# bowen-upenn/scene_graph_commonsense

Measured on AMD Instinct MI355X. Metric: ordered object-pairs/sec (relation head fwd+bwd), batch=8, N=64, higher is better.
Workload: dtype f16 fwd / bf16 bwd (f32 accumulate, f32 master weights); 1 GPU; VG PredCLS synthetic, 8 images x 64 objects per GPU = 32256 ordered pairs per GPU per step, from the raw minibatch; parallelism=dp1

## Files before the change

include/sgc_relhead.h:

```cpp
#ifndef SGC_RELHEAD_H
#define SGC_RELHEAD_H
#ifdef __cplusplus
extern "C" {
#endif


int sgc_pack_image_nhwc(const float* f0, int C0, const float* f1, int C1, void* x_out, int n_img, int HW, int XC, void* stream);

int sgc_conv1_tanh(const void* x, const void* w1r, const float* b1, void* a_img, int n_rows, int XC, void* stream);

int sgc_object_masked_maps(const void* a_img, const int* obj_img, const int* bbox, const void* cst, void* a_pad, int n_obj, int F, int D, void* stream);

int sgc_conv2_object(const void* a_pad, const void* w2r, const float* bias, void* out, int n_obj, void* stream);

int sgc_pair_expand(const void* U, const void* V, const int* sub_idx, const int* obj_idx, void* z_pad, int n_pairs, int out_elem, void* stream);

int sgc_pair_expand_dense(const void* U, const void* V, const int* img_ptr, const int* pid, int pid_ld, int n_img, int max_n,
                          void* z_pad_f16, void* z_pad_bf16, unsigned char* amz, void* stream);
int sgc_pair_expand_dense_windows(const void* U, const void* V, const int* img_ptr, const int* pid, int pid_ld, int n_img, int max_n,
                                  void* z_pad_f16, void* z_pad_bf16, unsigned char* amz, const int* pixel_rect, void* stream);

int sgc_conv3_relu_pool(const void* z_pad, const void* w3r, const float* b3, void* y, unsigned char* argmax, void* y_bf16, int n_pairs,
                        void* stream);

int sgc_shared_windows_count(const int* bbox, const int* sub_idx, const int* obj_idx, int n_pairs, int* count, int* pixel_rect,
                             void* stream);
int sgc_shared_windows_fill(const int* bbox, const int* sub_idx, const int* obj_idx, int n_pairs, const int* count_incl, int* gather,
                            void* stream);
int sgc_conv3_relu_pool_windows(const void* z_pad, const void* w3r, const float* b3, const int* gather, const int* gather_n,
                                int max_entries, void* y, unsigned char* argmax, void* y_bf16, void* stream);
int sgc_shared_windows_assemble(const int* bbox, const int* sub_idx, const int* obj_idx, int n_pairs, int n_obj, const void* y_obj,
                                const unsigned char* argmax_obj, const void* y_obj_bf16, void* y, unsigned char* argmax, void* y_bf16,
                                void* stream);

int sgc_conv2_regions_count(const int* bbox, int n_obj, int* count, void* stream);
int sgc_conv2_regions_fill(const int* bbox, int n_obj, const int* count_incl, int* gather, void* stream);
int sgc_conv2_object_regions(const void* a_pad, const void* w2r, const float* bias, const int* gather, const int* gather_n,
                             int max_entries, void* uv, void* stream);
int sgc_conv2_fill_background(const int* bbox, const int* obj_img, int n_obj, void* uv, void* stream);

int sgc_shared_windows_count3(const int* bbox, const int* sub_idx, const int* obj_idx, int n_pairs, int* count_all, int* count_conv,
                              int* count_linear, int* pixel_rect_conv, void* stream);
int sgc_shared_windows_fill_class(const int* bbox, const int* sub_idx, const int* obj_idx, int n_pairs, const int* count_incl, int* gather,
                                  int cls, void* stream);
int sgc_conv3_windows_raw(const void* z_pad, const void* w3r, const int* gather, const int* gather_n, int max_entries, float* raw,
                          void* stream);
int sgc_conv3_relu_pool_windows_wm_raw(const void* z_pad, const void* w3r, const float* b3, const int* gather, const int* gather_n,
                                       const int* dest, int max_entries, void* ywm, unsigned char* argmax, void* ywm_bf16, float* raw,
                                       int raw_first, void* stream);
int sgc_windows_linear_forward(const int* bbox, const int* sub_idx, const int* obj_idx, const int* obj_img, int n_obj, int n_real_pairs,
                               const int* gather_linear, const int* n_linear, int max_linear, const int* count_incl_all,
                               const int* dest_all, const float* raw, long n_object_entries, const float* b3, void* ywm, void* ywm_bf16,
                               unsigned char* argmax, int* dest_linear, void* stream);
int sgc_windows_linear_backward_objects(const int* bbox, const int* sub_idx, const int* obj_idx, const int* sub_ptr, const int* sub_list,
                                        const int* obj_ptr, const int* obj_list, int n_obj, int n_real_pairs, const int* gather_conv,
                                        int first_object_entry, int n_object_entries, const int* count_incl_all, const int* dest_all,
                                        const void* dywm, const unsigned char* argmax, void* dy3x, void* stream);
int sgc_windows_linear_backward_bg(const int* gather_linear, const int* dest_linear, const int* order, const int* segments, int n_img,
                                   const void* dywm, const unsigned char* argmax, void* dy3_bg_pad, float* bias_part, void* stream);

int sgc_shared_windows_assemble_bwd(const int* bbox, const int* sub_idx, const int* obj_idx, const int* sub_ptr, const int* sub_list,
                                    const int* obj_ptr, const int* obj_list, int n_obj, const void* dy, void* dy_obj, void* stream);
int sgc_windows_unpool(const void* dy, const unsigned char* argmax, const int* gather, const int* gather_n, const int* dest,
                       int entries_pad, void* dy3x, float* bias_part, int* n_parts, void* stream);
int sgc_windows_im2col(const void* z_pad_bf16, const int* gather, const int* gather_n, int entries_pad, void* zcol, void* stream);
int sgc_windows_wgrad(const void* dy3x, const void* zcol, float* slabs, int rows, int splits, int* n_slabs, void* stream);
int sgc_windows_wgrad_gather(const void* dy3x, const void* z_pad_bf16, const int* gather, float* slabs, int rows, int splits, int* n_slabs,
                             void* stream);
int sgc_windows_im2patch(const void* z_pad_bf16, const int* gather, const int* gather_n, int entries_pad, void* zpatch, void* stream);
int sgc_windows_im2patch_f16(const void* z_pad_f16, const int* gather, const int* gather_n, int entries_pad, void* zpatch, void* stream);
int sgc_windows_wgrad_patch(const void* dy3x, const void* zpatch, float* slabs, int rows, int splits, int* n_slabs, void* stream);
int sgc_windows_wgrad_patch_sparse(const void* dywm, const unsigned char* argmax, const int* gather, const int* dest, int n_entries,
                                   const void* zpatch, void* pack_ac, void* pack_ic, float* slabs, int splits, int* n_slabs, void* stream);
int sgc_windows_wgrad_gather_sparse(const void* dywm, const unsigned char* argmax, const int* gather, const int* dest, int n_entries,
                                    const void* z_pad_f16, void* pack_ac, void* pack_ic, float* slabs, int splits, int* n_slabs, void* stream);
int sgc_windows_im2patch_f16_from(const void* z_pad_f16, const int* gather, const int* gather_n, int e0, int entries, void* zpatch, void* stream);
int sgc_windows_dgrad_cols(const void* dy3x, const void* w3col, void* col, int rows, void* stream);
int sgc_windows_col2im(const void* col, const int* bbox, const int* sub_idx, const int* obj_idx, const int* count_incl, int n_pairs,
                       void* dz, void* stream);
int sgc_windows_dgrad_sparse_weights(const float* conv3_weight, void* w3sp, void* stream);
int sgc_windows_patch_sum2(const void* patch, int n16, const int* bbox, const int* sub_idx, const int* obj_idx, const int* count_incl, int n_pairs,
                           void* dz, void* stream);
int sgc_windows_patch_sum_objects2(const void* patch, int n16, const int* bbox, int n_obj, int n_real, const int* count_incl, void* dz, void* stream);
int sgc_windows_dgrad_sparse_pack(const void* dywm, const unsigned char* argmax, const int* gather, const int* dest, int n_sparse,
                                  void* pack_a, void* pack_i, float* bias_part, int* n_parts, void* stream);
int sgc_windows_dgrad_patches_sparse(const void* pack_a, const void* pack_i, int n_sparse, const void* w3sp, void* patch, void* stream);
int sgc_windows_unpool_from(const void* dy, const unsigned char* argmax, const int* gather, const int* gather_n, const int* dest, int entry0,
                            int entries_pad, void* dy3x, float* bias_part, int* n_parts, void* stream);
int sgc_windows_patch_slots(void);
int sgc_windows_dgrad_patches(const void* dy3x, const void* w3patch, void* patch, int entries, void* stream);
int sgc_windows_patch_sum(const void* patch, const int* bbox, const int* sub_idx, const int* obj_idx, const int* count_incl, int n_pairs,
                          void* dz, void* stream);
int sgc_windows_patch_sum_objects(const void* patch, const int* bbox, int n_obj, int n_real_pairs, const int* count_incl, void* dz, void* stream);
int sgc_pair_contract_windows(const void* dz, const unsigned char* amz, const int* ptr, const int* list, const int* pixel_rect,
                              const int* img_ptr, int role, int n_real_pairs, int n_obj, int n_img, int bg_maps, void* dU_pad, void* stream);
int sgc_shared_objects_count(const int* bbox, int n_obj, int* count, int* pixel_rect, void* stream);
int sgc_shared_objects_fill(const int* bbox, int n_obj, int n_real_pairs, const int* count_incl, int* gather, void* stream);
int sgc_shared_objects_fill_rows(const int* bbox, const int* obj_img, int n_obj, const int* goff, const void* y_bg, const void* y_bg_bf16,
                                 const unsigned char* argmax_bg, void* ywm, void* ywm_bf16, unsigned char* argmax_ps, void* stream);
int sgc_shared_objects_bg_grad(const int* bbox, const int* img_ptr, int n_obj, int n_img, const int* goff, const void* dywm, void* dy_bg,
                               void* stream);
int sgc_windows_col2im_objects(const void* col, const int* bbox, int n_obj, int n_real_pairs, const int* count_incl, void* dz, void* stream);

int sgc_conv3_relu_pool_wm(const void* z_pad, const void* w3r, const float* b3, const int* goff, void* ywm, unsigned char* argmax,
                           void* ywm_bf16, int n_pairs, void* stream);
int sgc_conv3_relu_pool_windows_wm(const void* z_pad, const void* w3r, const float* b3, const int* gather, const int* gather_n,
                                   const int* dest, int max_entries, void* ywm, unsigned char* argmax, void* ywm_bf16, void* stream);
int sgc_fc1_products_pitch(void);
int sgc_fc1_windows_gemm(const void* ywm, const void* w1p, const int* tile_group, float* owm, int rows, void* stream);
int sgc_fc1_integral(const float* owm, const int* goff, int n_pseudo, float* S, void* stream);
int sgc_fc1_own_rect_sums(const float* S, const int* bbox, int n_obj, float* own, void* stream);
int sgc_fc1_assemble(const float* S, const float* owm, const int* bbox, const int* sub_idx, const int* obj_idx, const int* count_incl,
                     const int* dest, int n_obj, const float* bias, int drop_enable, unsigned drop_seed, void* h1, int n_pairs,
                     const float* own_rect_sums , void* stream);
int sgc_fc1_assemble_ordered(const float* S, const float* owm, const int* bbox, const int* sub_idx, const int* obj_idx, const int* count_incl,
                             const int* dest, int n_obj, const float* bias, int drop_enable, unsigned drop_seed, void* h1, int n_pairs,
                             const float* own_rect_sums, const int* pair_order, void* stream);
int sgc_fc1_windows_gemm_x16(const void* ywm, const void* w1p, const int* tile_group, const int* goff, int n_pseudo, float* owm, void* oxh,
                             int rows, void* stream);
int sgc_fc1_assemble_x16(const float* S, const void* oxh, const int* bbox, const int* sub_idx, const int* obj_idx, const int* count_incl,
                         const int* dest, int n_obj, const float* bias, int drop_enable, unsigned drop_seed, void* h1, int n_pairs,
                         const float* own_rect_sums, const int* pair_order, void* stream);

int sgc_fc1_gsum(const void* dh1, const int* bbox, const int* sub_idx, const int* obj_idx, const int* sub_ptr, const int* sub_list,
                 const int* obj_ptr, const int* obj_list, const int* goff, int n_obj, void* gwm, void* stream);
int sgc_fc1_xrows(const void* dh1, const int* gather, const int* dest, int n_entries, const int* goff, const int* gend, void* gwm,
                  void* ywm_bf16, void* stream);
int sgc_fc1_windows_dgrad(const void* gwm, const void* w1pT, const int* tile_group, void* dywm, int rows, void* stream);
int sgc_fc1_windows_wgrad(const void* gwm, const void* ywm_bf16, const int* goff, float* dw, int rows, void* stream);

int sgc_window_rows_compact(const int* bbox, const int* obj_img, int n_obj, int n_img, const int* goff, int* prow, void* stream);
int sgc_window_rows_objects_compact(const int* codes, int n, const int* prow, int n_pairs, int* dest, void* stream);
int sgc_shared_objects_fill_argmax(const int* bbox, const int* obj_img, int n_obj, const unsigned char* argmax_bg, unsigned char* argmax_ps,
                                   void* stream);
int sgc_fc1_integral_rows(const float* owm, const int* prow, int n_pseudo, float* S, void* stream);
int sgc_fc1_gsum_groups(int n_obj, int n_img);
int sgc_fc1_gsum_compact(const void* dh1, const int* bbox, const int* sub_idx, const int* obj_idx, const int* sub_ptr, const int* sub_list,
                         const int* obj_ptr, const int* obj_list, const int* img_ptr, int n_img, const int* goff, const int* prow, int n_obj,
                         void* gwm, float* part, void* stream);
int sgc_shared_objects_bg_grad_compact(int n_img, const int* goff, const void* dywm, void* dy_bg, void* stream);

int sgc_fc1_relu(const void* y, const void* w1p, const float* b, void* h1, int n_pairs, int K, int drop_enable, unsigned drop_seed, void* stream);

int sgc_fc2_labels_relu(const void* h1, const void* w2m, const float* b, const float* lsub, const float* lobj, const int* sub_idx,
                        const int* obj_idx, float* p_out, int n_pairs, int drop_enable, unsigned drop_seed, void* stream);

int sgc_bayes_head(const float* p, const float* Wt, const float* bias, int n_pairs, int ng, int np, int ns, int hier, float T1, float T2,
                   float T3, float* rel, float* sup, float* conn, float* cand_conf, int* cand_pred, const unsigned char* iou_mask, void* stream);

int sgc_bayes_head_any(const float* h, const float* W, const float* bias, int M, int D, int ng, int np, int ns, float T1, float T2,
                       float T3, float* rel, float* sup, void* stream);
int sgc_bayes_head_any_bwd(const float* h, const float* W, const float* rel, const float* sup, const float* g_rel, const float* g_sup,
                           int M, int D, int ng, int np, int ns, float T1, float T2, float T3, float* dh, float* part, void* stream);
int sgc_bayes_head_any_wreduce(const float* part, int n_part, int D, float* out, void* stream);
int sgc_bayes_head_any_loss(const float* h, const float* W, const float* bias, const void* target, int target_is_int64,
                            const float* class_weight, int M, int D, int ng, int np, int ns, float T1, float T2, float T3, float* norm,
                            float* dz, double* loss_part, float* loss, void* stream);
int sgc_bayes_head_any_loss_bwd(const float* h, const float* W, const float* dz, const float* g, int M, int D, float* dh, float* part,
                                void* stream);
int sgc_bayes_head_any_candidates(const float* h, const float* W, const float* bias, int M, int D, int ng, int np, int ns, float T1,
                                  float T2, float T3, float* cand_conf, int* cand_pred, float* sup, void* stream);
int sgc_bayes_head_any_loss_cs(const float* h, const float* W, const float* bias, const void* target, int target_is_int64,
                               const float* class_weight, const void* subject_cat, const void* object_cat, int cat_is_int64,
                               const unsigned* aligned, const unsigned* violated, int C, int M, int D, int ng, int np, int ns, float T1,
                               float T2, float T3, float lambda_cs, float lambda_weak, float lambda_strong, float* norm, float* dz,
                               float* dir, unsigned char* flags, double* part, int* cnt_part, float* out, long long* counts,
                               void* stream);
int sgc_bayes_head_any_loss_cs_bwd(const float* h, const float* W, const float* dz, const float* dir, const unsigned char* flags,
                                   const float* coef, const float* g, int M, int D, int ng, int np, int ns, float* dh, float* part,
                                   void* stream);
int sgc_bayes_head_any_candidates_cs(const float* h, const float* W, const float* bias, const void* subject_cat, const void* object_cat,
                                     int cat_is_int64, const unsigned* aligned, const unsigned* violated, int C, int M, int D, int ng,
                                     int np, int ns, float T1, float T2, float T3, float* cand_conf, int* cand_pred, float* sup,
                                     void* stream);

int sgc_topk_per_image(const float* conf, const int* seg_ptr, int n_img, int K, int* out_idx, int* out_count, void* stream);

int sgc_scene_graph_topk(const float* cand_conf, const int* cand_pred, int rep, const float* cat_conf, const float* conn,
                         const unsigned char* mask, const unsigned char* included, const int* image_ptr, const int* pair_list,
                         const int* sub_idx, const int* obj_idx, const long* cats, const unsigned* aligned, const unsigned* violated,
                         int C, int R, int n_img, int K, int slot_major, int* out_pair, int* out_slot, int* out_pred, int* out_sub,
                         int* out_obj, float* out_score, int* out_count, int* out_finite, void* stream);

int sgc_recall_hits(const long* c_scat, const long* c_ocat, const long* c_pred, int n_pred, const float* c_sbox, const float* c_obox,
                    const int* keep_pos, const int* keep_cnt, int K, const int* t_row, const long* t_rel, const long* t_scat,
                    const long* t_ocat, const float* t_sbox, const float* t_obox, int n_targets, const unsigned char* equiv, int n_equiv,
                    int feature_size, double iou_thresh, int* hit, void* stream);

int sgc_related_topk(const long* c_scat, const long* c_ocat, const long* c_pred, const float* c_sbox, const float* c_obox,
                     const float* c_conf, int n_cand, const int* keep_pos, const int* keep_cnt, int K, int top_k, const int* t_ptr,
                     const long* t_scat, const long* t_ocat, const float* t_sbox, const float* t_obox, int n_img, int* out_pos,
                     int* out_rank, int* out_count, float* out_conf, void* stream);

int sgc_recall_accumulate(const int* out_pair, const int* out_pred, const int* out_sub, const int* out_obj, const int* out_count,
                          int n_img, int K, const int* cand_pred, int n_pred, const long* cats, const float* boxes, int n_obj,
                          const int* sub_idx, const int* obj_idx, const int* image, const int* directed,
                          const unsigned char* included, int n_pairs, const int* img_targets, const int* top_k, int n_k,
                          const unsigned* zero_shot, int C, int R, int feature_size, double iou_thresh, long* hits, long* hits_pc,
                          long* targets, long* targets_pc, long* zs_hits, long* zs_hits_pc, long* zs_targets, long* zs_targets_pc,
                          void* stream);

int sgc_recall_accumulate_targets(const int* out_pred, const int* out_sub, const int* out_obj, const int* out_count, int n_img, int K,
                                  const long* cats, const float* boxes, int n_obj, const int* t_image, const long* t_rel,
                                  const long* t_scat, const long* t_ocat, const float* t_sbox, const float* t_obox, int n_targets,
                                  const unsigned char* equiv, int n_equiv, const int* top_k, int n_k, const unsigned* zero_shot, int C,
                                  int R, int feature_size, double iou_thresh, long* hits, long* hits_pc, long* targets,
                                  long* targets_pc, long* zs_hits, long* zs_hits_pc, long* zs_targets, long* zs_targets_pc,
                                  void* stream);

int sgc_assign_pair_targets(const int* sub_idx, const int* obj_idx, const int* image, int n_pairs, const int* pid, int pid_ld,
                            const int* img_ptr, const long* cats, const float* boxes, int n_obj, const int* t_ptr, int n_img,
                            const long* t_rel, const long* t_scat, const long* t_ocat, const float* t_sbox, const float* t_obox,
                            int n_targets, const unsigned char* equiv, int n_equiv, int R, int feature_size, double iou_thresh,
                            int* directed, int* raw, int* matched, int* target_hit, void* stream);

int sgc_precision_accumulate(const int* out_pred, const int* out_sub, const int* out_obj, const int* out_count, int n_img, int K,
                             int n_rank, const int* image_ptr, const int* pair_list, const long* cats, const float* boxes, int n_obj,
                             const int* sub_idx, const int* obj_idx, const int* directed, const unsigned char* included, int n_pairs,
                             int R, int feature_size, double iou_thresh, long* ap, long* ap_union, long* num_ap, void* stream);

int sgc_overlap_filter(const int* bbox, const int* sub_idx, const int* obj_idx, unsigned char* out, int n_pairs, void* stream);

int sgc_commonsense_filter(const long* scat, const long* pred, const long* ocat, float* conf, int n, const unsigned* aligned,
                           const unsigned* violated, int C, int R, void* stream);

int sgc_commonsense_flags(const long* scat, const long* ocat, const int* cand_pred, int n_pairs, int n_cand, const unsigned* aligned,
                          const unsigned* violated, int C, int R, float* weak, float* strong, void* stream);


int sgc_scene_tables(const int* n_per_img, const int* img_ptr, const int* goff, int n_img, int max_n, int n_pairs, int n_obj, int pid_ld,
                     const int* rel_tri, const float* dir_tri, int* sub_idx, int* obj_idx, int* step, int* image, int* directed,
                     int* raw, int* pid, int* obj_ptr, int* sub_list, int* obj_list, int* obj_img, int* step_ptr, void* stream);

int sgc_bucket_place(const int* codes, int n, const int* sub_idx, const int* obj_img, int img_key, int n_keys, const int* base, int* out,
                     int* seg, int mode, void* stream);
long sgc_bucket_place_scratch_ints(int n, int n_keys);
int sgc_bucket_place_seg(const int* codes, int n, const int* sub_idx, const int* obj_img, int img_key, int n_keys, const int* base, int* out,
                         int* seg, int mode, int* scratch, long scratch_ints, void* stream);

int sgc_pseudo_pair_tables(const int* obj_img, int n_obj, int n_img, int n_pairs, int with_bg, int* ps_sub, int* ps_obj, int* bg_codes,
                           int* bg_n, void* stream);

int sgc_scan_rows(const int* in, int* out, int rows, int n, void* stream);

int sgc_window_rows_objects(const int* codes, int n, const int* goff, int n_pairs, int* dest, void* stream);
int sgc_window_rows_conv(const int* codes_conv, int n, const int* incl_conv, const int* incl_all, const int* dest_all, int* dest_conv,
                         void* stream);

int sgc_loss_coefficients(const int* step_ptr, int n_steps, const int* directed, const float* class_weight, int ng, int np, int hier,
                          double lambda_connectivity, double lambda_not_connected, int* tgt, float* coef_a, float* coef_b, float* coef_c,
                          float* conn_y, void* stream);

int sgc_connectivity_stats(const float* conn, const int* directed, const int* raw, const unsigned char* included, int n_pairs,
                           unsigned long long* out5, void* stream);

int sgc_label_vectors(const float* fc2_weight, int ld, int col0, const long* cats, const float* super_multihot, int n_obj, int C, int S,
                      float* lsub, float* lobj, void* stream);
int sgc_label_grads(const float* dlsub, const float* dlobj, const long* cats_sub, const long* cats_obj, const float* mh_sub,
                    const float* mh_obj, int n_obj, int C, int S, float* grad_fc2_weight, int ld, int col0, void* stream);


int sgc_pair_expand_train(const void* U, const void* V, const int* sub_idx, const int* obj_idx, void* z_pad_f16, void* z_pad_bf16,
                          unsigned char* amz, int n_pairs, void* stream);

int sgc_head_loss_bwd(const float* rel, const float* sup, const float* conn, const float* p, const int* tgt, const float* coef_a,
                      const float* coef_b, const float* coef_c, const float* conn_y, const float* W, int n_pairs, int ng, int np, int ns,
                      int hier, float T1, float T2, float T3, float drop_scale, float* dl, float* loss, void* dpre, const float* dp_extra,
                      const float* cs_coef, const float* cand_conf, const int* cand_pred, void* stream);
int sgc_head_bwd_upstream(const float* rel, const float* sup, const float* p, const float* g_rel, const float* g_sup, const float* g_conn,
                          const float* g_hidden, const float* W, int n_pairs, int ng, int np, int ns, int hier, float T1, float T2,
                          float T3, float drop_scale, float* dl, void* dpre, void* stream);
int sgc_head_wgrad(const float* dl, const float* p, float* part, int n_pairs, int chunk, void* stream);

int sgc_supcon_hierar(const float* F, const int* labels, int M, float temperature, float grad_scale, float* G, float* loss_rows,
                      float* dF, void* stream);

int sgc_slab_sum(const float* in, float* out, long n, int slabs, int accumulate, void* stream);
int sgc_fill_zero(void* ptr, long nbytes, void* stream);
int sgc_slab_sum_ld(const float* in, float* out, int rows, int cols, long ld_out, int slabs, void* stream);
int sgc_colsum(int elem, const void* X, float* part, long rows, int cols, int row_blocks, void* stream);
int sgc_segment_sum_rows(const void* X, const int* ptr, const int* list, float* out, int n_seg, int cols, void* stream);
int sgc_convert_f16_bf16(const void* in, void* out, long n, void* stream);
int sgc_transpose_cast(const float* src, void* dst, int out_kind, int na, int nb, long sa_s, long sb_s, long ss_i, long sa_d,
                       long sb_d, long ds_j, void* stream);
int sgc_permute_cast(const float* src, void* dst, int out_kind, int ndim, const int* dims, const long* src_strides, const long* dst_strides,
                     long src_off, long dst_off, void* stream);
int sgc_segment_cast(const float* src, void* dst, int out_kind, int rows, int cols, long src_row_stride, long src_col_stride, int n_seg,
                     const long* dst_off, const long* dst_ld, const long* src_off, void* stream);

int sgc_fc2_dgrad(const void* dpre, const void* w2mT, const void* h1, void* dh1, int n_pairs, float drop_scale, void* stream);
int sgc_fc2_wgrad(const void* dpre, const void* h1_bf16, float* slabs, int n_rows, int splits, int* n_slabs, void* stream);
int sgc_fc1_dgrad(const void* dh1, const void* w1pT, void* dy, int n_pairs, int K, void* stream);
int sgc_fc1_wgrad(const void* dh1, const void* y_bf16, float* dw, int n_rows, int K, void* stream);
int sgc_unpool_relu_bwd(const void* dy, const unsigned char* argmax, void* dy3_pad, float* dbias_part, int* n_parts, int n_pairs, void* stream);
int sgc_conv3_dgrad(const void* dy3_pad, const void* wd3, void* dz, int n_pairs, void* stream);
int sgc_conv3_dgrad_pooled(const void* dy, const unsigned char* argmax, const void* wd3, void* dz, int n_pairs, void* stream);
int sgc_conv3_wgrad(const void* dy3_pad, const void* z_pad_bf16, float* slabs, int n_pairs, int splits, int* n_slabs, void* stream);
int sgc_conv3_wgrad_sparse(const void* dy, const unsigned char* argmax, const void* z_pad_bf16, void* pack_ac, void* pack_ic,
                           float* slabs, int n_pairs, int splits, int* n_slabs, void* stream);
int sgc_unpool_relu_bwd_pack(const void* dy, const unsigned char* argmax, void* dy3_pad, float* dbias_part, int* n_parts,
                             void* pack_ac, void* pack_ic, int n_pairs, void* stream);
int sgc_pair_contract(const void* dz, const unsigned char* amz, const int* ptr, const int* list, void* dU_pad, int n_obj, void* stream);
int sgc_conv2_dgrad(const void* dU_pad, const void* wd2, void* da, int n_obj, void* stream);
int sgc_conv2_bwd_regions(const int* bbox, int n_real, int n_objx, int dilate, int* gather, int* n_out, void* stream);
int sgc_conv2_dgrad_regions(const void* dU_pad, const void* wd2, const int* gather, const int* gather_n, int max_entries, void* da,
                            void* stream);
int sgc_conv2_wgrad(const void* dU_pad, const void* a_pad_bf16, float* slabs, int n_obj, int splits, int* n_slabs, void* stream);
int sgc_object_masked_maps_bwd(const void* da, const int* img_ptr, const int* bbox, float* dA, float* dcst_part, int* n_parts, int n_img,
                               int F, int D, void* stream);
int sgc_tanh_bwd(const float* dA, const void* a_img, void* dpre, long n, void* stream);
int sgc_conv1_wgrad(const void* dpre, const void* x_bf16, float* slabs, int n_rows, int XC, int splits, int* n_slabs, void* stream);

int sgc_conv1_dgrad(const void* dpre_a, const void* wt_a, const void* dpre_b, const void* wt_b, float* out0, int C0, float* out1, int C1,
                    int n_img, int HW, int accumulate, void* stream);

int sgc_sgd_momentum_step(float* w, const float* g, float* momentum_buf, long n, float lr, float momentum, float weight_decay,
                          int first_step, void* stream);
int sgc_sgd_fc1_fused(float* w, const float* g_gemm_order, float* momentum_buf, int rows, float lr, float momentum, float weight_decay,
                      int first_step, void* w1p_f16, void* stream);
int sgc_sgd_momentum_multi(int n_tensors, float* const* w, const float* const* g, float* const* momentum_buf, const long* n, float lr,
                           float momentum, float weight_decay, unsigned first_mask, void* stream);

int sgc_detr_candidates(const float* logits, const float* boxes, const int* alp2fre, int n_img, int n_query, int C1, int num_classes,
                        int topk, float feature_size, int* cand_cat, float* cand_conf, float* cand_box, void* stream);
int sgc_nms_per_class(const int* cand_cat, const float* cand_conf, const float* cand_box, int n_img, int n_query, int topk,
                      double iou_threshold, int* out_slot, int* out_count, void* stream);
int sgc_match_boxes_top2(const float* pred_box, const int* pred_ptr, const float* tgt_box, const int* tgt_ptr, int n_img, int max_tgt,
                         int feature_size, int* top_idx, float* top_iou, void* stream);


int sgc_generic_conv1_tanh(const float* feat, const float* depth, long stride_feat, long stride_depth, const int* img, const int* box,
                           const float* w1, const float* b1, int n_pairs, int C, int F, float* a, void* stream);
int sgc_generic_conv3x3_relu_pool(const float* in, const float* w, const float* b, int n_pairs, int S, int Cin, int Cout, float* out,
                                  unsigned char* code, void* stream);
int sgc_generic_conv3x3_bwd(const float* in, const float* w, const float* dout, const unsigned char* code, int n_pairs, int S, int Cin, int Cout,
                            float* dpre, float* din, float* dw, float* db, void* stream);
int sgc_generic_fc1_relu(const float* y, const float* w1, const float* b1, int n_pairs, int Q, int C8, int dropout, unsigned seed, void* h1,
                         void* stream);
int sgc_generic_fc1_bwd(const void* dh1, const float* y, const float* w1, int n_pairs, int Q, int C8, float* dy, float* dw1, float* db1,
                        void* stream);
int sgc_generic_conv1_bwd(const float* feat, const float* depth, long stride_feat, long stride_depth, const int* img, const int* box, const float* a,
                          float* da, int n_pairs, int C, int F, float* dw1, float* db1, void* stream);
int sgc_generic_conv1_dgrad(const float* dpre1, const float* w1, const int* img, const int* box, int n_pairs, int C, int F, float* out0, int C0,
                            float* out1, int C1, int n_img, int accumulate, void* stream);

int sgc_dbg_gemm_nt(int elem, const void* A, const void* B, void* C, int M, int N, int K, long lda, long ldb, long ldc, const float* bias, void* stream);
int sgc_dbg_gemm_nt_ld(const void* A, const void* B, void* C, int M, int N, int K, long lda, long ldb, void* stream);
int sgc_dbg_conv_nt(int elem, const void* A, const void* B, void* C, int n_img, int lgS, int Cin, int N, const float* bias, void* stream);
int sgc_dbg_gemm_tn(int elem, const void* A, const void* B, float* C, int M, int N, int K, long lda, long ldb, int splits, int* slabs, void* stream);
int sgc_dbg_conv_tn(int elem, const void* A, const void* B, float* C, int M, int n_img, int lgS, int Cin, int splits, int* slabs, void* stream);
int sgc_dbg_tr_probe(const int* addr, short* out, void* stream);
int sgc_dbg_mfma_rate(float* out, int blocks, int iters, int mode, void* stream);
int sgc_dbg_smfmac_probe(const void* a, const void* b, const int* idx, float* c, int abid, void* stream);

#ifdef __cplusplus
}
#endif
#endif
```

scene_graph_commonsense_amd/csrc/capi_debug.hip:

```cpp
#include "gemm_nt.h"
#include "gemm_tn.h"

extern "C" {

int sgc_dbg_gemm_nt(int elem, const void* A, const void* B, void* C, int M, int N, int K,
                    long lda, long ldb, long ldc, const float* bias, void* stream) {
    NtParams p{};
    p.A = (const u16*)A; p.B = (const u16*)B; p.C = C; p.M = M; p.N = N; p.K = K;
    p.lda = lda; p.ldb = ldb; p.ldc = ldc; p.bias = bias;
    if (elem == ELEM_F16) return launch_gemm_nt<ELEM_F16, AMODE_PLAIN, EPI_STORE>(p, (hipStream_t)stream);
    return launch_gemm_nt<ELEM_BF16, AMODE_PLAIN, EPI_STORE>(p, (hipStream_t)stream);
}

int sgc_dbg_gemm_nt_ld(const void* A, const void* B, void* C, int M, int N, int K, long lda, long ldb, void* stream) {
    NtParams p{};
    p.A = (const u16*)A; p.B = (const u16*)B; p.C = C; p.M = M; p.N = N; p.K = K;
    p.lda = lda; p.ldb = ldb; p.ldc = N; p.epi_lds = 1;
    if ((N % 256) || (K % 64) || (lda % 8) || (ldb % 8)) return SGC_ERR_ARG;
    return launch_gemm_nt_pp<ELEM_BF16, EPI_STORE>(p, (hipStream_t)stream);
}

int sgc_dbg_conv_nt(int elem, const void* A, const void* B, void* C, int n_img, int lgS, int Cin, int N,
                    const float* bias, void* stream) {
    NtParams p{};
    p.A = (const u16*)A; p.B = (const u16*)B; p.C = C; p.M = n_img << (2 * lgS); p.N = N; p.K = 9 * Cin;
    p.ldb = 9L * Cin; p.ldc = N; p.lgS = lgS; p.Cin = Cin; p.bias = bias;
    if (elem == ELEM_F16) return launch_gemm_nt<ELEM_F16, AMODE_CONV, EPI_STORE>(p, (hipStream_t)stream);
    return launch_gemm_nt<ELEM_BF16, AMODE_CONV, EPI_STORE>(p, (hipStream_t)stream);
}

int sgc_dbg_gemm_tn(int elem, const void* A, const void* B, float* C, int M, int N, int K,
                    long lda, long ldb, int splits, int* slabs, void* stream) {
    TnParams p{};
    p.A = (const u16*)A; p.B = (const u16*)B; p.C = C; p.M = M; p.N = N; p.K = K;
    p.lda = lda; p.ldb = ldb; p.ldc = N; p.slab_stride = (long)M * N;
    int r = (elem == ELEM_F16) ? launch_gemm_tn<ELEM_F16, BMODE_PLAIN>(p, splits, slabs, (hipStream_t)stream)
                               : launch_gemm_tn<ELEM_BF16, BMODE_PLAIN>(p, splits, slabs, (hipStream_t)stream);
    return r;
}

int sgc_dbg_conv_tn(int elem, const void* A, const void* B, float* C, int M, int n_img, int lgS, int Cin,
                    int splits, int* slabs, void* stream) {
    TnParams p{};
    p.A = (const u16*)A; p.B = (const u16*)B; p.C = C; p.M = M; p.N = 9 * Cin; p.K = n_img << (2 * lgS);
    p.lda = M; p.ldc = 9L * Cin; p.slab_stride = (long)M * 9 * Cin; p.lgS = lgS; p.Cin = Cin;
    int r = (elem == ELEM_F16) ? launch_gemm_tn<ELEM_F16, BMODE_CONV>(p, splits, slabs, (hipStream_t)stream)
                               : launch_gemm_tn<ELEM_BF16, BMODE_CONV>(p, splits, slabs, (hipStream_t)stream);
    return r;
}

__global__ void tr_probe_kernel(const int* addr, short* out) {
    __shared__ __attribute__((aligned(16))) short lds[4096];
    for (int i = threadIdx.x; i < 4096; i += 64) lds[i] = (short)i;
    __syncthreads();
    const s16x4 v = __builtin_amdgcn_ds_read_tr16_b64_v4i16(
        (__attribute__((address_space(3))) s16x4*)((char*)lds + addr[threadIdx.x]));
    for (int j = 0; j < 4; ++j) out[threadIdx.x * 4 + j] = v[j];
}
int sgc_dbg_tr_probe(const int* addr, short* out, void* stream) {
    SGC_LAUNCH(tr_probe_kernel, dim3(1), dim3(64), 0, (hipStream_t)stream, addr, out);
    SGC_CHECK_LAUNCH();
    return SGC_OK;
}

__global__ void smfmac_probe_kernel(const u16* a, const u16* b, const int* idx, float* c, int abid) {
    typedef __bf16 bf16x8_t __attribute__((ext_vector_type(8)));
    typedef __bf16 bf16x16_t __attribute__((ext_vector_type(16)));
    const int l = threadIdx.x;
    bf16x8_t av; bf16x16_t bv;
    for (int i = 0; i < 8; ++i) { u16 t = a[l * 8 + i]; av[i] = __builtin_bit_cast(__bf16, t); }
    for (int i = 0; i < 16; ++i) { u16 t = b[l * 16 + i]; bv[i] = __builtin_bit_cast(__bf16, t); }
    f32x16 acc;
    for (int r = 0; r < 16; ++r) acc[r] = 0.f;
    if (abid == 0) acc = __builtin_amdgcn_smfmac_f32_32x32x32_bf16(av, bv, acc, idx[l], 0, 0);
    else if (abid == 1) acc = __builtin_amdgcn_smfmac_f32_32x32x32_bf16(av, bv, acc, idx[l], 0, 1);
    else acc = __builtin_amdgcn_smfmac_f32_32x32x32_bf16(av, bv, acc, idx[l], 1, 0);
    for (int r = 0; r < 16; ++r) c[l * 16 + r] = acc[r];
}
int sgc_dbg_smfmac_probe(const void* a, const void* b, const int* idx, float* c, int abid, void* stream) {
    SGC_LAUNCH(smfmac_probe_kernel, dim3(1), dim3(64), 0, (hipStream_t)stream, (const u16*)a, (const u16*)b, idx, c, abid);
    SGC_CHECK_LAUNCH();
    return SGC_OK;
}

}
template <int mode>
__global__ __launch_bounds__(512, 2) void mfma_rate_kernel(float* out, int iters) {
    typedef __bf16 bf16x8_t __attribute__((ext_vector_type(8)));
    typedef __bf16 bf16x16_t __attribute__((ext_vector_type(16)));
    f32x16 acc[8];
    for (int i = 0; i < 8; ++i) for (int r = 0; r < 16; ++r) acc[i][r] = 0.f;
    bf16x8_t a; bf16x16_t b;
    for (int i = 0; i < 8; ++i) a[i] = (__bf16)(float)(threadIdx.x * 0.001f + i);
    for (int i = 0; i < 16; ++i) b[i] = (__bf16)(float)(threadIdx.x * 0.002f + i);
    const bf16x8_t b8 = __builtin_shufflevector(b, b, 0, 1, 2, 3, 4, 5, 6, 7);
    const int idx = 0x4444;
    for (int it = 0; it < iters; ++it) {
        if (mode == 0) {
#pragma unroll
            for (int i = 0; i < 8; ++i) acc[i] = __builtin_amdgcn_mfma_f32_32x32x16_bf16(a, b8, acc[i], 0, 0, 0);
        } else {
#pragma unroll
            for (int i = 0; i < 8; ++i) acc[i] = __builtin_amdgcn_smfmac_f32_32x32x32_bf16(a, b, acc[i], idx, 0, 0);
        }
    }
    float s = 0.f;
    for (int i = 0; i < 8; ++i) for (int r = 0; r < 16; ++r) s += acc[i][r];
    if (s == 12345.678f) out[0] = s;
}
extern "C" {
int sgc_dbg_mfma_rate(float* out, int blocks, int iters, int mode, void* stream) {
    if (mode == 0) SGC_LAUNCH(mfma_rate_kernel<0>, dim3(blocks), dim3(512), 0, (hipStream_t)stream, out, iters);
    else SGC_LAUNCH(mfma_rate_kernel<1>, dim3(blocks), dim3(512), 0, (hipStream_t)stream, out, iters);
    SGC_CHECK_LAUNCH();
    return SGC_OK;
}

}
```

scene_graph_commonsense_amd/csrc/gemm_nt.h:

```cpp
#pragma once
#include "common.h"
#include <type_traits>

enum { AMODE_PLAIN = 0, AMODE_CONV = 1, AMODE_CONV_GATHER = 2 };
enum { EPI_STORE = 0, EPI_BIAS_TANH = 1, EPI_BIAS_RELU = 2, EPI_POOL = 3, EPI_FC2 = 4, EPI_RELUMASK = 5, EPI_STORE_F32 = 6,
       EPI_STORE_F32T = 7 };

struct NtParams {
    const u16* A; const u16* B; void* C;
    int M, N, K;
    long lda, ldb, ldc;
    int lgS, Cin;
    const float* bias;
    const u16* mask_src;
    const float* lsub; const float* lobj; const int* sub_idx; const int* obj_idx;
    unsigned char* argmax;
    u16* C2;
    float scale;
    unsigned drop_seed; int drop_enable;
    int tiles_m, tiles_n;
    int epi_lds;
    int halo_walk;
    int patch_aligned;
    const u16* Apool; const unsigned char* Acode;
    const int* gather; const int* gather_n;
    const int* dest;
    const int* wm_goff;
    float* raw; int raw_first;
    const int* tile_group; long group_stride;
    u16* Cx; int x_first;
    long seg_stride; int seg_bpad, seg_split;
};

template <int ELEM>
__device__ __forceinline__ f32x16 mfma32(s16x8 a, s16x8 b, f32x16 c) {
    if constexpr (ELEM == ELEM_F16) {
        return __builtin_amdgcn_mfma_f32_32x32x16_f16(__builtin_bit_cast(f16x8, a), __builtin_bit_cast(f16x8, b), c, 0, 0, 0);
    } else {
        return __builtin_amdgcn_mfma_f32_32x32x16_bf16(__builtin_bit_cast(bf16x8, a), __builtin_bit_cast(bf16x8, b), c, 0, 0, 0);
    }
}

__device__ __forceinline__ long conv_row_base(int m, int lgS, int Cin) {
    const int S = 1 << lgS;
    const int img = m >> (2 * lgS);
    const int ml = m & (S * S - 1);
    const int W = ml >> 2, q = ml & 3;
    const int py = W >> (lgS - 1), px = W & ((S >> 1) - 1);
    const int y = 2 * py + (q >> 1), x = 2 * px + (q & 1);
    return ((long)(img * (S + 2) + y) * (S + 2) + x) * Cin;
}

template <int ELEM, int EPI, int TM, int TN, bool GATHER = false>
__device__ __forceinline__ void nt_epilogue(const NtParams& p, f32x16 (&acc)[TM][TN], int m0, int n0, int wr, int wc, int lane, int m_limit = -1) {
    const int M = GATHER ? m_limit : p.M;
    const int h = lane >> 5, cl = lane & 31;
#pragma unroll
    for (int i = 0; i < TM; ++i) {
#pragma unroll
        for (int j = 0; j < TN; ++j) {
            const int col = n0 + wc * TN * 32 + j * 32 + cl;
            const int rbase = m0 + wr * TM * 32 + i * 32;
            const float bias = p.bias ? p.bias[col] : 0.f;
            if constexpr (EPI == EPI_POOL) {
                u16* out = reinterpret_cast<u16*>(p.C);
#pragma unroll
                for (int w = 0; w < 4; ++w) {
                    float v = acc[i][j][4 * w];
                    int am = 0;
#pragma unroll
                    for (int q = 1; q < 4; ++q) {
                        const float t = acc[i][j][4 * w + q];
                        if (t > v) { v = t; am = q; }
                    }
                    v += bias;
                    const int prow = (rbase >> 2) + 2 * w + h;
                    if (prow * 4 < M) {
                        long arow = prow, yrow = prow;
                        if constexpr (GATHER) {
                            arow = p.gather[prow]; yrow = p.dest ? p.dest[prow] : arow;
                            if (p.raw && prow >= p.raw_first) {
#pragma unroll
                                for (int q = 0; q < 4; ++q) p.raw[((long)(prow - p.raw_first) * 4 + q) * p.ldc + col] = acc[i][j][4 * w + q];
                            }
                        }
                        else if (p.wm_goff) yrow = p.wm_goff[prow & 63] + (prow >> 6);
                        if (!(v > 0.f)) { v = 0.f; am = 4; }
                        out[yrow * p.ldc + col] = to_elem<ELEM>(v);
                        if (p.C2) p.C2[yrow * p.ldc + col] = f32_to_bf16_bits(v);
                        if (p.argmax) p.argmax[arow * p.ldc + col] = (unsigned char)am;
                    }
                }
            } else {
#pragma unroll
                for (int r = 0; r < 16; ++r) {
                    const int row = rbase + (r & 3) + 8 * (r >> 2) + 4 * h;
                    if (row >= M) continue;
                    float v = acc[i][j][r];
                    long o = (long)row * p.ldc + col;
                    if constexpr (GATHER && EPI == EPI_STORE)
                        o = ((long)p.gather[row >> 2] * 4 + (row & 3)) * p.ldc + col;
                    if constexpr (EPI == EPI_STORE) {
                        reinterpret_cast<u16*>(p.C)[o] = to_elem<ELEM>(v + bias);
                    } else if constexpr (EPI == EPI_STORE_F32) {
                        reinterpret_cast<float*>(p.C)[o] = v + bias;
                    } else if constexpr (EPI == EPI_BIAS_TANH) {
                        reinterpret_cast<u16*>(p.C)[o] = to_elem<ELEM>(tanhf(v + bias));
                    } else if constexpr (EPI == EPI_BIAS_RELU) {
                        v = fmaxf(v + bias, 0.f);
                        if (p.drop_enable) v = dropout_keep(p.drop_seed, (uint32_t)(row * p.N + col)) ? v * p.scale : 0.f;
                        reinterpret_cast<u16*>(p.C)[o] = to_elem<ELEM>(v);
                    } else if constexpr (EPI == EPI_FC2) {
                        v += bias + p.lsub[(long)p.sub_idx[row] * p.N + col] + p.lobj[(long)p.obj_idx[row] * p.N + col];
                        v = fmaxf(v, 0.f);
                        if (p.drop_enable) v = dropout_keep(p.drop_seed, (uint32_t)(row * p.N + col)) ? v * p.scale : 0.f;
                        reinterpret_cast<float*>(p.C)[o] = v;
                    } else if constexpr (EPI == EPI_RELUMASK) {
                        const float f = from_elem<ELEM_F16>(p.mask_src[o]);
                        reinterpret_cast<u16*>(p.C)[o] = to_elem<ELEM>(f > 0.f ? v * p.scale : 0.f);
                    }
                }
            }
        }
    }
}

__device__ __forceinline__ void nt_epilogue_f32t(const NtParams& p, f32x16 (&acc)[4][2], int m0, int n0, int wr, int wc, int lane) {
    const int h = lane >> 5, cl = lane & 31;
    float* out = reinterpret_cast<float*>(p.C);
    if (!out) return;
    const int g_first = p.Cx ? p.wm_goff[p.tile_group[m0 >> 8]] + p.x_first : 0;
#pragma unroll
    for (int i = 0; i < 4; ++i) {
        const int row = m0 + wr * 128 + i * 32 + cl;
        if (row >= p.M) continue;
        const bool xrow = p.Cx && row >= g_first;
#pragma unroll
        for (int j = 0; j < 2; ++j) {
#pragma unroll
            for (int rq = 0; rq < 4; ++rq) {
                const int col = n0 + wc * 64 + j * 32 + 8 * rq + 4 * h;
                f32x4 v = {acc[i][j][4 * rq], acc[i][j][4 * rq + 1], acc[i][j][4 * rq + 2], acc[i][j][4 * rq + 3]};
                if (p.bias) {
                    const f32x4 b = *reinterpret_cast<const f32x4*>(p.bias + col);
                    v += b;
                }
                if (xrow) {
                    uint2 hv;
                    hv.x = (unsigned)f32_to_f16_bits(v[0]) | ((unsigned)f32_to_f16_bits(v[1]) << 16);
                    hv.y = (unsigned)f32_to_f16_bits(v[2]) | ((unsigned)f32_to_f16_bits(v[3]) << 16);
                    *reinterpret_cast<uint2*>(p.Cx + (long)row * p.N + col) = hv;
                    continue;
                }
                f32x4* dst = reinterpret_cast<f32x4*>(out + (long)row * p.ldc + col);
                *dst = v;
            }
        }
    }
}

__device__ __forceinline__ void supertile_map(int id, int tiles_m, int tiles_n, int& tm, int& tn) {
    constexpr int GS = 16;
    const int a = id / (GS * tiles_n);
    const int hm = min(GS, tiles_m - a * GS);
    const int id2 = id - a * GS * tiles_n;
    const int sn = (tiles_n + GS - 1) / GS;
    const int b = min(id2 / (hm * GS), sn - 1);
    const int id3 = id2 - b * hm * GS;
    const int wn = min(GS, tiles_n - b * GS);
    tm = a * GS + id3 / wn;
    tn = b * GS + id3 % wn;
}

__device__ __forceinline__ void supertile_map_g(int id, int tiles_m, int tiles_n, int GM, int GN, int& tm, int& tn) {
    const int a = id / (GM * tiles_n);
    const int hm = min(GM, tiles_m - a * GM);
    const int id2 = id - a * GM * tiles_n;
    const int sn = (tiles_n + GN - 1) / GN;
    const int b = min(id2 / (hm * GN), sn - 1);
    const int id3 = id2 - b * hm * GN;
    const int wn = min(GN, tiles_n - b * GN);
    tm = a * GM + id3 / wn;
    tn = b * GN + id3 % wn;
}

constexpr int EPI_LDS_PITCH = 128;
constexpr int EPI_LDS_BYTES = 8 * 128 * EPI_LDS_PITCH;
template <int ELEM, bool MASK = false>
__device__ __forceinline__ void nt_epilogue_store16(const NtParams& p, f32x16 (&acc)[4][2], int m0, int n0, int wr, int wc, int lane,
                                                    int wid, char* smem) {
    __syncthreads();
    char* reg = smem + wid * (128 * EPI_LDS_PITCH);
    const int h = lane >> 5, cl = lane & 31;
    const bool odd = cl & 1;
#pragma unroll
    for (int i = 0; i < 4; ++i) {
#pragma unroll
        for (int j = 0; j < 2; ++j) {
            const int col = n0 + wc * 64 + j * 32 + cl;
            const float bias = p.bias ? p.bias[col] : 0.f;
#pragma unroll
            for (int rp = 0; rp < 8; ++rp) {
                float v0 = acc[i][j][2 * rp] + bias, v1 = acc[i][j][2 * rp + 1] + bias;
                if constexpr (MASK) { v0 *= p.scale; v1 *= p.scale; }
                const float recv = __shfl_xor(odd ? v0 : v1, 1);
                const int r0 = ((2 * rp) & 3) + 8 * ((2 * rp) >> 2) + 4 * h;
                const float flo = odd ? recv : v0, fhi = odd ? v1 : recv;
                unsigned packed;
                if constexpr (ELEM == ELEM_BF16) packed = f32x2_to_bf16x2_bits(flo, fhi);
                else packed = (unsigned)to_elem<ELEM>(flo) | ((unsigned)to_elem<ELEM>(fhi) << 16);
                const int row = i * 32 + r0 + (odd ? 1 : 0);
                *reinterpret_cast<unsigned*>(reg + row * EPI_LDS_PITCH + (((j * 32 + (cl & ~1)) * 2) ^ ((row & 1) << 6))) = packed;
            }
        }
    }
    __builtin_amdgcn_wave_barrier();
    u16* out = reinterpret_cast<u16*>(p.C);
    const int c8 = lane & 7, rsub = lane >> 3;
#pragma unroll
    for (int it = 0; it < 16; ++it) {
        const int rowl = it * 8 + rsub;
        uint4 v = *reinterpret_cast<const uint4*>(reg + rowl * EPI_LDS_PITCH + ((c8 * 16) ^ ((rowl & 1) << 6)));
        const int row = m0 + wr * 128 + rowl;
        if (row < p.M) {
            const long o = (long)row * p.ldc + n0 + wc * 64 + c8 * 8;
            if constexpr (MASK) {
                const uint4 f = *reinterpret_cast<const uint4*>(p.mask_src + o);
                const u16* fh = reinterpret_cast<const u16*>(&f);
                u16* vh = reinterpret_cast<u16*>(&v);
#pragma unroll
                for (int k = 0; k < 8; ++k)
                    if (!(from_elem<ELEM_F16>(fh[k]) > 0.f)) vh[k] = 0;
            }
            *reinterpret_cast<uint4*>(out + o) = v;
        }
    }
}

template <int ELEM, int AMODE, int EPI, int WR, int WC, int TM, int TN>
__global__ __launch_bounds__(WR * WC * 64, 2) void gemm_nt_kernel(const NtParams p) {
    extern __shared__ __attribute__((aligned(16))) char smem[];
    constexpr int NW = WR * WC;
    constexpr int BM = WR * TM * 32, BN = WC * TN * 32;
    constexpr int A_BYTES = BM * 128, B_BYTES = BN * 128, BUF_BYTES = A_BYTES + B_BYTES;
    constexpr int AI = BM / (8 * NW), BI = BN / (8 * NW);
    const int tid = threadIdx.x, lane = tid & 63;
    const int wid = __builtin_amdgcn_readfirstlane(tid >> 6);
    int tm, tn;
    supertile_map(blockIdx.x, p.tiles_m, p.tiles_n, tm, tn);
    const int m0 = tm * BM, n0 = tn * BN;
    int Mlim = p.M;
    if constexpr (AMODE == AMODE_CONV_GATHER) {
        Mlim = min(p.M, 4 * *p.gather_n);
        if (m0 >= Mlim) return;
    }

    const int lrow = lane >> 3, cpos = lane & 7;
    const u16* a_ptr[AI];
    const u16* b_ptr[BI];
#pragma unroll
    for (int i = 0; i < AI; ++i) {
        const int row = wid * AI * 8 + i * 8 + lrow;
        const int chunk = cpos ^ ((row >> 1) & 7);
        int m = m0 + row; if (m > Mlim - 1) m = Mlim - 1;
        if constexpr (AMODE == AMODE_CONV_GATHER) m = p.gather[m >> 2] * 4 + (m & 3);
        if constexpr (AMODE != AMODE_PLAIN) a_ptr[i] = p.A + conv_row_base(m, p.lgS, p.Cin) + chunk * 8;
        else a_ptr[i] = p.A + (long)m * p.lda + chunk * 8;
    }
#pragma unroll
    for (int i = 0; i < BI; ++i) {
        const int row = wid * BI * 8 + i * 8 + lrow;
        const int chunk = cpos ^ ((row >> 1) & 7);
        b_ptr[i] = p.B + (long)(n0 + row) * p.ldb + chunk * 8;
    }
    const int Wp = (1 << p.lgS) + 2;

    auto stage = [&](int buf, int kt) {
        long aoff;
        if constexpr (AMODE != AMODE_PLAIN) {
            const int cc = kt / 9, tap = kt - cc * 9;
            const int ky = tap / 3, kx = tap - 3 * ky;
            aoff = (long)(ky * Wp + kx) * p.Cin + (cc << 6);
        } else {
            aoff = (long)kt << 6;
        }
        const long boff = (long)kt << 6;
        char* abase = smem + buf * BUF_BYTES + wid * (AI * 1024);
        char* bbase = smem + buf * BUF_BYTES + A_BYTES + wid * (BI * 1024);
#pragma unroll
        for (int i = 0; i < AI; ++i)
            __builtin_amdgcn_global_load_lds(GLB_PTR(a_ptr[i] + aoff), LDS_PTR(abase + i * 1024), 16, 0, 0);
#pragma unroll
        for (int i = 0; i < BI; ++i)
            __builtin_amdgcn_global_load_lds(GLB_PTR(b_ptr[i] + boff), LDS_PTR(bbase + i * 1024), 16, 0, 0);
    };

    const int wr = wid / WC, wc = wid % WC;
    const int kh = lane >> 5;
    int a_off[TM], a_sw[TM], b_off[TN], b_sw[TN];
#pragma unroll
    for (int i = 0; i < TM; ++i) {
        const int ra = wr * TM * 32 + i * 32 + (lane & 31);
        a_off[i] = ra * 128; a_sw[i] = (ra >> 1) & 7;
    }
#pragma unroll
    for (int i = 0; i < TN; ++i) {
        const int rb = wc * TN * 32 + i * 32 + (lane & 31);
        b_off[i] = rb * 128; b_sw[i] = (rb >> 1) & 7;
    }
    f32x16 acc[TM][TN];
#pragma unroll
    for (int i = 0; i < TM; ++i)
#pragma unroll
        for (int j = 0; j < TN; ++j)
#pragma unroll
            for (int r = 0; r < 16; ++r) acc[i][j][r] = 0.f;

    const int nk = p.K >> 6;
    stage(0, 0);
    for (int kt = 0; kt < nk; ++kt) {
        asm volatile("s_waitcnt vmcnt(0)" ::: "memory");
        __syncthreads();
        if (kt + 1 < nk) stage((kt + 1) & 1, kt + 1);
        const char* ab = smem + (kt & 1) * BUF_BYTES;
        const char* bb = ab + A_BYTES;
#pragma unroll
        for (int ks = 0; ks < 4; ++ks) {
            const int c = ks * 2 + kh;
            s16x8 af[TM], bf[TN];
#pragma unroll
            for (int i = 0; i < TM; ++i) af[i] = *reinterpret_cast<const s16x8*>(ab + a_off[i] + ((c ^ a_sw[i]) << 4));
#pragma unroll
            for (int i = 0; i < TN; ++i) bf[i] = *reinterpret_cast<const s16x8*>(bb + b_off[i] + ((c ^ b_sw[i]) << 4));
#pragma unroll
            for (int i = 0; i < TM; ++i)
#pragma unroll
                for (int j = 0; j < TN; ++j) acc[i][j] = mfma32<ELEM>(af[i], bf[j], acc[i][j]);
        }
    }

    if constexpr (EPI == EPI_STORE && TM == 4 && TN == 2 && WR * WC == 8) {
        if (p.epi_lds) { nt_epilogue_store16<ELEM>(p, acc, m0, n0, wr, wc, lane, wid, smem); return; }
    }
    if constexpr (AMODE == AMODE_CONV_GATHER) nt_epilogue<ELEM, EPI, TM, TN, true>(p, acc, m0, n0, wr, wc, lane, Mlim);
    else nt_epilogue<ELEM, EPI, TM, TN>(p, acc, m0, n0, wr, wc, lane);
}

template <int ELEM, int AMODE, int EPI, int WR, int WC, int TM, int TN>
static int launch_gemm_nt_cfg(NtParams p, hipStream_t stream) {
    constexpr int BM = WR * TM * 32, BN = WC * TN * 32;
    constexpr int LDS0 = 2 * (BM + BN) * 128;
    constexpr int LDS = (EPI == EPI_STORE && TM == 4 && TN == 2 && WR * WC == 8 && LDS0 < EPI_LDS_BYTES) ? EPI_LDS_BYTES : LDS0;
    p.tiles_m = (p.M + BM - 1) / BM;
    p.tiles_n = p.N / BN;
    auto kern = gemm_nt_kernel<ELEM, AMODE, EPI, WR, WC, TM, TN>;
    (void)hipFuncSetAttribute(reinterpret_cast<const void*>(kern), hipFuncAttributeMaxDynamicSharedMemorySize, LDS);
    SGC_LAUNCH(kern, dim3((unsigned)(p.tiles_m * p.tiles_n)), dim3(WR * WC * 64), LDS, stream, p);
    SGC_CHECK_LAUNCH();
    return SGC_OK;
}


#include "gemm_nt_pp.h"

template <int ELEM, int AMODE, int EPI>
static int launch_gemm_nt(NtParams p, hipStream_t stream) {
    static_assert(AMODE == AMODE_PLAIN || AMODE == AMODE_CONV, "gathered rows have their own launchers");
    if (p.M <= 0) return SGC_OK;
    if ((p.K & 63) || (p.N & 127) || p.K <= 0) return SGC_ERR_ARG;
    if (AMODE == AMODE_CONV && ((p.Cin & 63) || p.K != 9 * p.Cin)) return SGC_ERR_ARG;
    p.epi_lds = 1;
    const bool big = (p.N % 256) == 0 && (long)p.M * p.N >= 256L * 256 * 256;
    if constexpr (AMODE == AMODE_CONV && (EPI == EPI_POOL || EPI == EPI_STORE)) {
        if (big && p.lgS == 4 && (p.M % 256) == 0) return launch_conv16_halo_pp<ELEM, EPI>(p, stream);
    }
    if (big) {
        if constexpr (AMODE == AMODE_PLAIN) return launch_gemm_nt_pp<ELEM, EPI>(p, stream);
        else return launch_gemm_nt_cfg<ELEM, AMODE, EPI, 2, 4, 4, 2>(p, stream);
    }
    return launch_gemm_nt_cfg<ELEM, AMODE, EPI, 2, 2, 2, 2>(p, stream);
}
```

scene_graph_commonsense_amd/csrc/gemm_nt_pp.h:

```cpp
#pragma once

#define SGC_WAIT_VM(n) asm volatile("s_waitcnt vmcnt(" #n ")" ::: "memory")
#define SGC_WAIT_LGKM0() asm volatile("s_waitcnt lgkmcnt(0)" ::: "memory")
#define SGC_PP_BARRIER()                                       \
    do {                                                       \
        __builtin_amdgcn_sched_barrier(0);                     \
        __builtin_amdgcn_s_barrier();                          \
        __builtin_amdgcn_sched_barrier(0);                     \
    } while (0)

__device__ __forceinline__ void buf_load_lds16(const void* base, int voff, int soff, void* lds) {
    const __amdgpu_buffer_rsrc_t r = __builtin_amdgcn_make_buffer_rsrc(const_cast<void*>(base), 0, 0x7fffffff, 0x00020000);
    __builtin_amdgcn_raw_ptr_buffer_load_lds(r, LDS_PTR(lds), 16, voff, soff, 0, 0);
}

__device__ __forceinline__ void xcd_patch_map(int id, int tiles_m, int tiles_n, int& tm, int& tn, int gm = 4, int gn = 8) {
    const int nb = tiles_m * tiles_n, q = nb >> 3, r = nb & 7, x = id & 7;
    const int lin = (x < r ? x * (q + 1) : r * (q + 1) + (x - r) * q) + (id >> 3);
    supertile_map_g(lin, tiles_m, tiles_n, gm, gn, tm, tn);
}

__host__ __device__ __forceinline__ int xcd_patch_gn(int tiles_n) { return tiles_n >= 8 ? 8 : (tiles_n >= 4 ? 4 : (tiles_n >= 2 ? 2 : 1)); }
static inline int xcd_patch_grid(int tiles_m, int tiles_n) {
    const int gn = xcd_patch_gn(tiles_n), gm = 32 / gn;
    const int npatch = ((tiles_m + gm - 1) / gm) * ((tiles_n + gn - 1) / gn);
    return ((npatch + 7) / 8) * 8 * 32;
}
__device__ __forceinline__ bool xcd_patch_map_aligned(int id, int tiles_m, int tiles_n, int& tm, int& tn) {
    const int gn = xcd_patch_gn(tiles_n), gm = 32 / gn;
    const int sn = (tiles_n + gn - 1) / gn, npatch = ((tiles_m + gm - 1) / gm) * sn;
    const int x = id & 7, j = id >> 3;
    const int patch = (j >> 5) * 8 + x, w = j & 31;
    if (patch >= npatch) return false;
    const int a = patch / sn, b = patch - a * sn;
    const int wn = min(gn, tiles_n - b * gn);
    tm = a * gm + w / wn;
    tn = b * gn + w % wn;
    return tm < tiles_m && w < gm * wn;
}

template <int ELEM, bool GATHER>
__device__ __forceinline__ void nt_epilogue_pool16(const NtParams& p, f32x16 (&acc)[4][2], int m0, int n0, int wr, int wc, int lane,
                                                   int wid, char* smem, int m_limit);
template <int ELEM, int EPI, int ACG = 0, int SEG = 0>
__global__ __launch_bounds__(512, 2) void gemm_nt_pp_kernel(const NtParams p) {
    extern __shared__ __attribute__((aligned(16))) char smem[];
    constexpr int HT = 16384;
    const int tid = threadIdx.x, lane = tid & 63;
    const int wid = __builtin_amdgcn_readfirstlane(tid >> 6);
    const int wr = wid >> 2, wc = wid & 3;
    int tm, tn;
    if constexpr (SEG) {
        xcd_patch_map(blockIdx.x, p.tiles_m, p.tiles_n, tm, tn, 16, 2);
    } else if (p.patch_aligned) {
        if (!xcd_patch_map_aligned(blockIdx.x, p.tiles_m, p.tiles_n, tm, tn)) return;
    } else {
        xcd_patch_map(blockIdx.x, p.tiles_m, p.tiles_n, tm, tn);
    }
    const int m0 = tm * 256;
    int n0 = tn * 256, n_tile = tn, Kloc = p.K, seg_py = 0, seg_px = 0, seg_ny = 1, seg_nx = 1, seg_c0 = 0;
    long ldb = p.ldb, b_off = 0;
    if constexpr (SEG) {
        const int slot = tn >> 1;
        int pp = 0, part = 0;
        if (p.seg_split) {
            int acc = 0;
            for (pp = 0; pp < 16; ++pp) {
                const int wdt = (((pp >> 2) == 1 || (pp >> 2) == 2) && ((pp & 3) == 1 || (pp & 3) == 2)) ? 2 : 1;
                if (slot < acc + wdt) { part = slot - acc; break; }
                acc += wdt;
            }
        } else {
            pp = slot;
        }
        n_tile = tn & 1;
        n0 = slot * 512 + n_tile * 256;
        seg_py = pp >> 2; seg_px = pp & 3;
        auto cnt1 = [](int c) { return (c == 0 || c == 3) ? 1 : 2; };
        seg_ny = cnt1(seg_py); seg_nx = cnt1(seg_px);
        const int ncomb = seg_ny * seg_nx;
        seg_c0 = (p.seg_split && ncomb == 4) ? 2 * part : 0;
        Kloc = ((p.seg_split && ncomb == 4) ? 2 : ncomb) * 1024;
        ldb = ncomb * 1024 + p.seg_bpad;
        for (int j = 0; j < pp; ++j) b_off += 512L * (1024 * (cnt1(j >> 2) * cnt1(j & 3)) + p.seg_bpad);
        b_off += seg_c0 * 1024;
    }
    int Mlim = p.M;
    long img0 = 0;
    if constexpr (ACG) {
        Mlim = min(p.M, 4 * *p.gather_n);
        if (m0 >= Mlim) return;
        img0 = p.gather[m0 >> 2] >> (2 * p.lgS - 2);
    }
    const int SP = (1 << p.lgS) + 2;
    const long img_elems = (long)SP * SP * p.Cin;

    const int lrow = lane >> 3, cpos = lane & 7;
    const u16* const a_blk = ACG ? p.A + img0 * img_elems : p.A + (long)m0 * p.lda;
    const u16* const b_blk = p.B + b_off + (long)(n_tile * 256) * ldb + (p.tile_group ? (long)p.tile_group[tm] * p.group_stride : 0L);
    int voff[4][2];
#pragma unroll
    for (int q = 0; q < 2; ++q) {
        const int r = (wid * 2 + q) * 8 + lrow;
        const int chunk = (cpos ^ ((r >> 1) & 7)) << 3;
#pragma unroll
        for (int h = 0; h < 2; ++h) {
            int m = (r >> 6) * 128 + h * 64 + (r & 63);
            if (m0 + m > Mlim - 1) m = Mlim - 1 - m0;
            if constexpr (ACG) {
                const int mg = m0 + m;
                const int mv = p.gather[mg >> 2] * 4 + (mg & 3);
                voff[h ? 3 : 0][q] = (int)((conv_row_base(mv, p.lgS, p.Cin) - img0 * img_elems + chunk) * 2);
            } else {
                voff[h ? 3 : 0][q] = (int)((m * p.lda + chunk) * 2);
            }
            const int n = (r >> 5) * 64 + h * 32 + (r & 31);
            voff[1 + h][q] = (int)((n * ldb + chunk) * 2);
        }
    }
    auto stage = [&](int kind, int t) __attribute__((always_inline)) {
        char* base = smem + (((t & 1) << 2) + kind) * HT + wid * 2048;
        const u16* g = (kind == 0 || kind == 3) ? a_blk : b_blk;
        int soff = t << 7;
        if constexpr (ACG) {
            if (kind == 0 || kind == 3) {
                const int cc = t / 9, tap = t - cc * 9;
                const int ky = tap / 3, kx = tap - 3 * ky;
                soff = ((ky * SP + kx) * p.Cin + (cc << 6)) * 2;
            }
        }
        if constexpr (SEG) {
            if (kind == 0 || kind == 3) {
                const int c = seg_c0 + (t >> 4);
                const int cy = seg_nx == 2 ? (c >> 1) : c, cx = seg_nx == 2 ? (c & 1) : 0;
                const int qy = seg_ny == 1 ? (seg_py == 3) : cy, qx = seg_nx == 1 ? (seg_px == 3) : cx;
                g = a_blk + (long)(qy * 2 + qx) * p.seg_stride;
                soff = (t & 15) << 7;
            }
        }
        buf_load_lds16(g, voff[kind][0], soff, base);
        buf_load_lds16(g, voff[kind][1], soff, base + 1024);
    };

    const int l31 = lane & 31, kh = lane >> 5, sw = (l31 >> 1) & 7;
    int ko[4];
#pragma unroll
    for (int ks = 0; ks < 4; ++ks) ko[ks] = ((ks * 2 + kh) ^ sw) << 4;
    const int a_rd = (wr * 64 + l31) * 128, b_rd = (wc * 32 + l31) * 128;
    s16x8 af[2][4], bf[2][4];
    auto read_a = [&](int h, int par) __attribute__((always_inline)) {
        const char* base = smem + ((par << 2) + (h ? 3 : 0)) * HT + a_rd;
#pragma unroll
        for (int i = 0; i < 2; ++i)
#pragma unroll
            for (int ks = 0; ks < 4; ++ks) af[i][ks] = *reinterpret_cast<const s16x8*>(base + i * 4096 + ko[ks]);
    };
    auto read_b = [&](int par) __attribute__((always_inline)) {
#pragma unroll
        for (int h = 0; h < 2; ++h) {
            const char* base = smem + ((par << 2) + 1 + h) * HT + b_rd;
#pragma unroll
            for (int ks = 0; ks < 4; ++ks) bf[h][ks] = *reinterpret_cast<const s16x8*>(base + ko[ks]);
        }
    };

    f32x16 acc[4][2];
#pragma unroll
    for (int i = 0; i < 4; ++i)
#pragma unroll
        for (int j = 0; j < 2; ++j)
#pragma unroll
            for (int r = 0; r < 16; ++r) acc[i][j][r] = 0.f;
    auto half = [&](int a) __attribute__((always_inline)) {
        __builtin_amdgcn_sched_barrier(0);
#pragma unroll
        for (int ks = 0; ks < 4; ++ks)
#pragma unroll
            for (int i = 0; i < 2; ++i)
#pragma unroll
                for (int j = 0; j < 2; ++j) {
                    if constexpr (EPI == EPI_STORE_F32T) acc[2 * a + i][j] = mfma32<ELEM>(bf[j][ks], af[i][ks], acc[2 * a + i][j]);
                    else acc[2 * a + i][j] = mfma32<ELEM>(af[i][ks], bf[j][ks], acc[2 * a + i][j]);
                }
        SGC_PP_BARRIER();
    };
#define SGC_PP_CLOSE(STEADY)                                   \
    do {                                                       \
        if (STEADY) SGC_WAIT_VM(8); else SGC_WAIT_VM(0);       \
        SGC_WAIT_LGKM0();                                      \
        SGC_PP_BARRIER();                                      \
    } while (0)

    const int nk = Kloc >> 6;
    stage(0, 0); stage(1, 0); stage(2, 0); stage(3, 0);
    if (nk > 1) { stage(0, 1); stage(1, 1); stage(2, 1); SGC_WAIT_VM(8); } else SGC_WAIT_VM(0);
    __builtin_amdgcn_s_barrier();
    if (wr == 1) __builtin_amdgcn_s_barrier();

    auto tile = [&](int t, int par, auto steady_c) __attribute__((always_inline)) {
        constexpr bool STEADY = decltype(steady_c)::value;
        read_a(0, par); read_b(par);
        if (t + 1 < nk) stage(3, t + 1);
        SGC_PP_CLOSE(STEADY);
        half(0);
        read_a(1, par);
        if (STEADY) { stage(0, t + 2); stage(1, t + 2); stage(2, t + 2); }
        SGC_PP_CLOSE(STEADY);
        half(1);
    };
    int t = 0;
#pragma unroll 1
    for (; t + 2 < nk; ++t) tile(t, t & 1, std::true_type{});
#pragma unroll 1
    for (; t < nk; ++t) tile(t, t & 1, std::false_type{});
    if (wr == 0) __builtin_amdgcn_s_barrier();

    bool stored = false;
    if constexpr (EPI == EPI_STORE && !ACG) {
        if (p.epi_lds) { nt_epilogue_store16<ELEM>(p, acc, m0, n0, wr, wc, lane, wid, smem); stored = true; }
    }
    if constexpr (EPI == EPI_RELUMASK && !ACG) {
        if (p.epi_lds && !p.bias && (p.ldc & 7) == 0) { nt_epilogue_store16<ELEM, true>(p, acc, m0, n0, wr, wc, lane, wid, smem); stored = true; }
    }
    if (stored) {
    } else if constexpr (EPI == EPI_STORE_F32T) {
        static_assert(!ACG, "transposed f32 tile: plain rows only");
        nt_epilogue_f32t(p, acc, m0, n0, wr, wc, lane);
    }
    else if constexpr (ACG && EPI == EPI_POOL) {
        if (p.epi_lds) nt_epilogue_pool16<ELEM, true>(p, acc, m0, n0, wr, wc, lane, wid, smem, Mlim);
        else nt_epilogue<ELEM, EPI, 4, 2, true>(p, acc, m0, n0, wr, wc, lane, Mlim);
    }
    else if constexpr (ACG) nt_epilogue<ELEM, EPI, 4, 2, true>(p, acc, m0, n0, wr, wc, lane, Mlim);
    else nt_epilogue<ELEM, EPI, 4, 2>(p, acc, m0, n0, wr, wc, lane);
}

template <int ELEM, int EPI>
static int launch_gemm_nt_pp_conv_gather(NtParams p, hipStream_t stream) {
    constexpr int LDS = 8 * 16384;
    if ((p.lgS != 4 && p.lgS != 5) || (p.Cin & 63) || p.K != 9 * p.Cin || (p.N & 255)) return SGC_ERR_ARG;
    p.tiles_m = (p.M + 255) / 256;
    p.tiles_n = p.N / 256;
    p.patch_aligned = 0;
    if (EPI == EPI_POOL) p.epi_lds = 1;
    auto kern = gemm_nt_pp_kernel<ELEM, EPI, 1>;
    (void)hipFuncSetAttribute(reinterpret_cast<const void*>(kern), hipFuncAttributeMaxDynamicSharedMemorySize, LDS);
    SGC_LAUNCH(kern, dim3((unsigned)(p.tiles_m * p.tiles_n)), dim3(512), LDS, stream, p);
    SGC_CHECK_LAUNCH();
    return SGC_OK;
}

template <int ELEM>
static int launch_gemm_nt_pp_seg(NtParams p, hipStream_t stream) {
    constexpr int LDS = EPI_LDS_BYTES;
    p.tiles_m = (p.M + 255) / 256;
    p.tiles_n = p.N / 256;
    p.epi_lds = 1;
    auto kern = gemm_nt_pp_kernel<ELEM, EPI_STORE, 0, 1>;
    (void)hipFuncSetAttribute(reinterpret_cast<const void*>(kern), hipFuncAttributeMaxDynamicSharedMemorySize, LDS);
    p.patch_aligned = 0;
    SGC_LAUNCH(kern, dim3((unsigned)(p.tiles_m * p.tiles_n)), dim3(512), LDS, stream, p);
    SGC_CHECK_LAUNCH();
    return SGC_OK;
}

template <int ELEM, int EPI>
static int launch_gemm_nt_pp(NtParams p, hipStream_t stream) {
    constexpr int LDS = (EPI == EPI_STORE) ? EPI_LDS_BYTES : 8 * 16384;
    p.tiles_m = (p.M + 255) / 256;
    p.tiles_n = p.N / 256;
    auto kern = gemm_nt_pp_kernel<ELEM, EPI>;
    (void)hipFuncSetAttribute(reinterpret_cast<const void*>(kern), hipFuncAttributeMaxDynamicSharedMemorySize, LDS);
    const int grid_aligned = xcd_patch_grid(p.tiles_m, p.tiles_n);
    const int nb = p.tiles_m * p.tiles_n;
    p.patch_aligned = (nb >= 1024 && (nb & 255) != 0 && grid_aligned * 10 <= nb * 11) ? 1 : 0;
    SGC_LAUNCH(kern, dim3((unsigned)(p.patch_aligned ? grid_aligned : p.tiles_m * p.tiles_n)), dim3(512), LDS, stream, p);
    SGC_CHECK_LAUNCH();
    return SGC_OK;
}


constexpr int POOL_EPI_PY = 128, POOL_EPI_PA = 64;
constexpr int POOL_EPI_WAVE_BYTES = 32 * POOL_EPI_PY * 2 + 32 * POOL_EPI_PA;
template <int ELEM, bool GATHER>
__device__ __forceinline__ void nt_epilogue_pool16(const NtParams& p, f32x16 (&acc)[4][2], int m0, int n0, int wr, int wc, int lane,
                                                   int wid, char* smem, int m_limit) {
    __syncthreads();
    char* ty = smem + wid * POOL_EPI_WAVE_BYTES;
    char* tb = ty + 32 * POOL_EPI_PY;
    char* ta = tb + 32 * POOL_EPI_PY;
    const int h = lane >> 5, cl = lane & 31;
#pragma unroll
    for (int i = 0; i < 4; ++i)
#pragma unroll
        for (int j = 0; j < 2; ++j) {
            const int colw = j * 32 + cl;
            const float bias = p.bias ? p.bias[n0 + wc * 64 + colw] : 0.f;
#pragma unroll
            for (int w = 0; w < 4; ++w) {
                float v = acc[i][j][4 * w];
                int am = 0;
#pragma unroll
                for (int q = 1; q < 4; ++q) {
                    const float t = acc[i][j][4 * w + q];
                    if (t > v) { v = t; am = q; }
                }
                v += bias;
                if (!(v > 0.f)) { v = 0.f; am = 4; }
                const int row = i * 8 + 2 * w + h;
                if constexpr (GATHER) {
                    const int prow = (m0 >> 2) + wr * 32 + row;
                    if (p.raw && prow >= p.raw_first && prow * 4 < m_limit) {
#pragma unroll
                        for (int q = 0; q < 4; ++q) p.raw[((long)(prow - p.raw_first) * 4 + q) * p.ldc + n0 + wc * 64 + colw] = acc[i][j][4 * w + q];
                    }
                }
                *reinterpret_cast<u16*>(ty + row * POOL_EPI_PY + colw * 2) = to_elem<ELEM>(v);
                if (p.C2) *reinterpret_cast<u16*>(tb + row * POOL_EPI_PY + colw * 2) = f32_to_bf16_bits(v);
                if (p.argmax) *reinterpret_cast<unsigned char*>(ta + row * POOL_EPI_PA + colw) = (unsigned char)am;
            }
        }
    __builtin_amdgcn_wave_barrier();
    const long prow0 = ((long)m0 >> 2) + wr * 32;
    const int c8 = lane & 7, r8 = lane >> 3;
    u16* out = reinterpret_cast<u16*>(p.C);
#pragma unroll
    for (int it = 0; it < 4; ++it) {
        const int row = it * 8 + r8;
        long orow = prow0 + row;
        if constexpr (GATHER) {
            if (orow * 4 >= m_limit) continue;
            orow = p.dest ? p.dest[orow] : p.gather[orow];
        } else if (p.wm_goff) orow = p.wm_goff[orow & 63] + (orow >> 6);
        const long o = orow * p.ldc + n0 + wc * 64 + c8 * 8;
        *reinterpret_cast<uint4*>(out + o) = *reinterpret_cast<const uint4*>(ty + row * POOL_EPI_PY + c8 * 16);
        if (p.C2) *reinterpret_cast<uint4*>(p.C2 + o) = *reinterpret_cast<const uint4*>(tb + row * POOL_EPI_PY + c8 * 16);
    }
    if (p.argmax) {
        const int c4 = lane & 3, r16 = lane >> 2;
#pragma unroll
        for (int it = 0; it < 2; ++it) {
            const int row = it * 16 + r16;
            long arow = prow0 + row;
            if constexpr (GATHER) {
                if (arow * 4 >= m_limit) continue;
                arow = p.gather[arow];
            }
            *reinterpret_cast<uint4*>(p.argmax + arow * p.ldc + n0 + wc * 64 + c4 * 16) =
                *reinterpret_cast<const uint4*>(ta + row * POOL_EPI_PA + c4 * 16);
        }
    }
}

template <int ELEM, int EPI, int ASRC = 0>
__global__ __launch_bounds__(512, 2) void conv16_halo_pp_kernel(const NtParams p) {
    extern __shared__ __attribute__((aligned(16))) char smem[];
    constexpr int A_BYTES = 328 * 128;
    constexpr int HT = 16384;
    char* const abuf0 = smem;
    char* const bbuf0 = smem + 2 * A_BYTES;
    const int tid = threadIdx.x, lane = tid & 63;
    const int wid = __builtin_amdgcn_readfirstlane(tid >> 6);
    const int wr = wid >> 2, wc = wid & 3;
    int img, tn;
    if (p.halo_walk) {
        const int nb = p.tiles_m * p.tiles_n, q = nb >> 3, r = nb & 7, x = blockIdx.x & 7;
        const int lin = (x < r ? x * (q + 1) : r * (q + 1) + (x - r) * q) + (blockIdx.x >> 3);
        img = lin / p.tiles_n; tn = lin - img * p.tiles_n;
    } else {
        img = blockIdx.x / p.tiles_n; tn = blockIdx.x - img * p.tiles_n;
    }
    const int m0 = img * 256, n0 = tn * 256;
    const int Cin = p.Cin;

    const int lrow = lane >> 3, cpos = lane & 7;
    int a_off[6];
#pragma unroll
    for (int i = 0; i < 6; ++i) {
        int r = (wid + 8 * i) * 8 + lrow;
        if (r > 323) r = 323;
        const int py = r / 18, px = r - py * 18;
        const int f = ((px >> 1) + 4 * (py & 1)) & 7;
        a_off[i] = r * Cin + ((cpos ^ f) << 3);
    }
    const u16* const a_img = ASRC ? p.A : p.A + (long)img * (324L * Cin);
    const int npiece = ASRC ? 0 : ((wid == 0) ? 6 : 5);
    auto stage_a_piece = [&](int i, int cc) __attribute__((always_inline)) {
        buf_load_lds16(a_img, a_off[i] * 2, cc << 7, abuf0 + (cc & 1) * A_BYTES + (wid + 8 * i) * 1024);
    };
    char* const pscr = smem + 2 * A_BYTES + 4 * HT;
    const int pw = tid >> 3, pg = tid & 7;
    const u16* const apool_img = ASRC ? p.Apool + (long)img * 64 * Cin : nullptr;
    const unsigned char* const acode_img = ASRC ? p.Acode + (long)img * 64 * Cin : nullptr;
    const int pool_voff = (pw * Cin + pg * 8) * 2;
    const int pool_coff = (wid * 16 + (lane >> 2)) * Cin + (lane & 3) * 16;
    const int npool = (wid < 4) ? 2 : 1;
    auto pool_dma = [&](int cc) __attribute__((always_inline)) {
        buf_load_lds16(apool_img, pool_voff, cc << 7, pscr + wid * 1024);
        if (wid < 4) buf_load_lds16(acode_img, pool_coff, cc << 6, pscr + 8192 + wid * 1024);
    };
    auto pool_scatter_q = [&](int cc, int q) __attribute__((always_inline)) {
        char* ab = abuf0 + (cc & 1) * A_BYTES;
        const uint4 pool_v = *reinterpret_cast<const uint4*>(pscr + tid * 16);
        const uint2 pool_c = *reinterpret_cast<const uint2*>(pscr + 8192 + pw * 64 + pg * 8);
        const u16* vh = reinterpret_cast<const u16*>(&pool_v);
        const unsigned char* ch = reinterpret_cast<const unsigned char*>(&pool_c);
        const int wy = pw >> 3, wx = pw & 7;
        const unsigned qq = (unsigned)q * 0x01010101u;
        const unsigned x0 = pool_c.x ^ qq, x1 = pool_c.y ^ qq;
        const unsigned m0 = ~(((x0 & 0x7f7f7f7fu) + 0x7f7f7f7fu) | x0) & 0x80808080u;
        const unsigned m1 = ~(((x1 & 0x7f7f7f7fu) + 0x7f7f7f7fu) | x1) & 0x80808080u;
        auto lanes = [](unsigned m, int e) __attribute__((always_inline)) {
            const unsigned lo = (unsigned)__builtin_amdgcn_sbfe(m, 8 * e + 7, 1), hi = (unsigned)__builtin_amdgcn_sbfe(m, 8 * e + 15, 1);
            return (lo & 0x0000ffffu) | (hi & 0xffff0000u);
        };
        uint4 o;
        o.x = pool_v.x & lanes(m0, 0); o.y = pool_v.y & lanes(m0, 2); o.z = pool_v.z & lanes(m1, 0); o.w = pool_v.w & lanes(m1, 2);
        (void)vh; (void)ch;
        const int py = 2 * wy + (q >> 1) + 1, px = 2 * wx + (q & 1) + 1;
        const int f = ((px >> 1) + 4 * (py & 1)) & 7;
        *reinterpret_cast<uint4*>(ab + (py * 18 + px) * 128 + ((pg ^ f) << 4)) = o;
    };
    auto pool_scatter = [&](int cc) __attribute__((always_inline)) {
#pragma unroll
        for (int q = 0; q < 4; ++q) pool_scatter_q(cc, q);
    };
    const u16* const b_blk = p.B + (long)n0 * p.ldb;
    int b_voff[2][2];
#pragma unroll
    for (int q = 0; q < 2; ++q) {
        const int r = (wid * 2 + q) * 8 + lrow;
        const int chunk = (cpos ^ ((r >> 1) & 7)) << 3;
#pragma unroll
        for (int h = 0; h < 2; ++h) b_voff[h][q] = (int)((((r >> 5) * 64 + h * 32 + (r & 31)) * p.ldb + chunk) * 2);
    }
    auto stage_b = [&](int step) __attribute__((always_inline)) {
        char* base = bbuf0 + ((step & 1) * 2) * HT + wid * 2048;
#pragma unroll
        for (int h = 0; h < 2; ++h) {
            buf_load_lds16(b_blk, b_voff[h][0], step << 7, base + h * HT);
            buf_load_lds16(b_blk, b_voff[h][1], step << 7, base + h * HT + 1024);
        }
    };

    const int l31 = lane & 31, kh = lane >> 5;
    int a_row[4], a_px[4], a_py[4];
#pragma unroll
    for (int i = 0; i < 4; ++i) {
        const int m = wr * 128 + i * 32 + l31;
        const int W = m >> 2, q = m & 3;
        a_py[i] = 2 * (W >> 3) + (q >> 1);
        a_px[i] = 2 * (W & 7) + (q & 1);
        a_row[i] = a_py[i] * 18 + a_px[i];
    }
    const int bsw = (l31 >> 1) & 7;
    int bko[4];
#pragma unroll
    for (int ks = 0; ks < 4; ++ks) bko[ks] = ((ks * 2 + kh) ^ bsw) << 4;
    const int b_rd = (wc * 32 + l31) * 128;
    s16x8 af[2][4], bf[2][4];
    auto read_a = [&](int h, int cc, int ky, int kx) __attribute__((always_inline)) {
        const char* ab = abuf0 + (cc & 1) * A_BYTES;
#pragma unroll
        for (int i = 0; i < 2; ++i) {
            const int ii = 2 * h + i;
            const char* rowp = ab + (a_row[ii] + ky * 18 + kx) * 128;
            const int f = (((a_px[ii] + kx) >> 1) + 4 * ((a_py[ii] + ky) & 1)) & 7;
#pragma unroll
            for (int ks = 0; ks < 4; ++ks) af[i][ks] = *reinterpret_cast<const s16x8*>(rowp + (((ks * 2 + kh) ^ f) << 4));
        }
    };
    auto read_b = [&](int step) __attribute__((always_inline)) {
#pragma unroll
        for (int h = 0; h < 2; ++h) {
            const char* base = bbuf0 + ((step & 1) * 2 + h) * HT + b_rd;
#pragma unroll
            for (int ks = 0; ks < 4; ++ks) bf[h][ks] = *reinterpret_cast<const s16x8*>(base + bko[ks]);
        }
    };

    f32x16 acc[4][2];
#pragma unroll
    for (int i = 0; i < 4; ++i)
#pragma unroll
        for (int j = 0; j < 2; ++j)
#pragma unroll
            for (int r = 0; r < 16; ++r) acc[i][j][r] = 0.f;
    auto half = [&](int a) __attribute__((always_inline)) {
        __builtin_amdgcn_sched_barrier(0);
#pragma unroll
        for (int ks = 0; ks < 4; ++ks)
#pragma unroll
            for (int i = 0; i < 2; ++i)
#pragma unroll
                for (int j = 0; j < 2; ++j) acc[2 * a + i][j] = mfma32<ELEM>(af[i][ks], bf[j][ks], acc[2 * a + i][j]);
        SGC_PP_BARRIER();
    };

    const int ncc = Cin >> 6;
    const int nsteps = ncc * 9;
    if constexpr (ASRC) {
        pool_dma(0);
        for (int i = tid; i < 2 * A_BYTES / 16; i += 512)
            *reinterpret_cast<uint4*>(abuf0 + i * 16) = make_uint4(0, 0, 0, 0);
        SGC_WAIT_VM(0);
        __syncthreads();
        pool_scatter(0);
        stage_b(0);
        if (nsteps > 1) { stage_b(1); SGC_WAIT_VM(4); } else SGC_WAIT_VM(0);
        SGC_WAIT_LGKM0();
    } else {
#pragma unroll
        for (int i = 0; i < 6; ++i)
            if (i < npiece) stage_a_piece(i, 0);
        stage_b(0);
        if (nsteps > 1) { stage_b(1); SGC_WAIT_VM(4); } else SGC_WAIT_VM(0);
    }
    __builtin_amdgcn_s_barrier();
    if (wr == 1) __builtin_amdgcn_s_barrier();

    int step = 0;
    for (int cc = 0; cc < ncc; ++cc) {
        const bool more_cc = cc + 1 < ncc;
#pragma unroll 1
        for (int tap = 0; tap < 9; ++tap, ++step) {
            const int ky = tap / 3, kx = tap - 3 * ky;
            read_a(0, cc, ky, kx); read_b(step);
            SGC_WAIT_LGKM0();
            SGC_PP_BARRIER();
            half(0);
            read_a(1, cc, ky, kx);
            if constexpr (ASRC) {
                if (step + 2 < nsteps) {
                    stage_b(step + 2);
                    if (more_cc && tap == 0) {
                        pool_dma(cc + 1);
                        if (npool == 2) SGC_WAIT_VM(6); else SGC_WAIT_VM(5);
                    } else SGC_WAIT_VM(4);
                } else SGC_WAIT_VM(0);
                if (more_cc && tap == 2) pool_scatter(cc + 1);

            } else if (step + 2 < nsteps) {
                stage_b(step + 2);
                if (more_cc && tap < npiece) {
                    switch (tap) {
                        case 0: stage_a_piece(0, cc + 1); break;
                        case 1: stage_a_piece(1, cc + 1); break;
                        case 2: stage_a_piece(2, cc + 1); break;
                        case 3: stage_a_piece(3, cc + 1); break;
                        case 4: stage_a_piece(4, cc + 1); break;
                        default: stage_a_piece(5, cc + 1); break;
                    }
                    SGC_WAIT_VM(5);
                } else SGC_WAIT_VM(4);
            } else SGC_WAIT_VM(0);
            SGC_WAIT_LGKM0();
            SGC_PP_BARRIER();
            half(1);
        }
    }
    if (wr == 0) __builtin_amdgcn_s_barrier();

    if constexpr (EPI == EPI_STORE) {
        if (p.epi_lds) { nt_epilogue_store16<ELEM>(p, acc, m0, n0, wr, wc, lane, wid, smem); return; }
    }
    if constexpr (EPI == EPI_POOL) {
        if (p.epi_lds) { nt_epilogue_pool16<ELEM, false>(p, acc, m0, n0, wr, wc, lane, wid, smem, 0); return; }
    }
    nt_epilogue<ELEM, EPI, 4, 2>(p, acc, m0, n0, wr, wc, lane);
}

template <int ELEM, int EPI>
static int launch_conv16_halo_pp(NtParams p, hipStream_t stream) {
    constexpr int LDS0 = 2 * 328 * 128 + 4 * 16384;
    constexpr int LDS = (EPI == EPI_STORE && LDS0 < EPI_LDS_BYTES) ? EPI_LDS_BYTES : LDS0;
    constexpr int LDS_POOLED = LDS0 + 64 * 128 + 64 * 64;
    p.tiles_m = p.M / 256;
    p.tiles_n = p.N / 256;
    {
        p.halo_walk = (long)p.K * 512 > (3L << 20) ? 1 : 0;
    }
    if constexpr (ELEM == ELEM_BF16 && EPI == EPI_STORE) {
        if (p.Apool) {
            auto kern = conv16_halo_pp_kernel<ELEM, EPI, 1>;
            (void)hipFuncSetAttribute(reinterpret_cast<const void*>(kern), hipFuncAttributeMaxDynamicSharedMemorySize, LDS_POOLED);
            SGC_LAUNCH(kern, dim3((unsigned)(p.tiles_m * p.tiles_n)), dim3(512), LDS_POOLED, stream, p);
            SGC_CHECK_LAUNCH();
            return SGC_OK;
        }
    }
    auto kern = conv16_halo_pp_kernel<ELEM, EPI>;
    (void)hipFuncSetAttribute(reinterpret_cast<const void*>(kern), hipFuncAttributeMaxDynamicSharedMemorySize, LDS);
    SGC_LAUNCH(kern, dim3((unsigned)(p.tiles_m * p.tiles_n)), dim3(512), LDS, stream, p);
    SGC_CHECK_LAUNCH();
    return SGC_OK;
}
```

scene_graph_commonsense_amd/csrc/kernels_dgrad_sp.hip:

```cpp
#include "common.h"
#include "gemm_nt.h"
#include "gemm_tn.h"

typedef __bf16 bf16x8_sp __attribute__((ext_vector_type(8)));
typedef __bf16 bf16x16_sp __attribute__((ext_vector_type(16)));
typedef short s16x16_sp_t __attribute__((ext_vector_type(16)));

static inline int grid_cap_sp(long items, long per_block, int cap) {
    long b = (items + per_block - 1) / per_block;
    if (b > cap) b = cap;
    if (b < 1) b = 1;
    return (int)b;
}

struct NtSpParams {
    const u16* Ac;
    const unsigned* Ic;
    const u16* B;
    u16* C;
    int entries;
    int tiles_m;
};

__host__ __device__ __forceinline__ int nt_sp_slot_set(int slot, int* pp_out = nullptr, int* part_out = nullptr) {
    int acc = 0, pp = 0, part = 0;
    for (pp = 0; pp < 16; ++pp) {
        const int wdt = (((pp >> 2) == 1 || (pp >> 2) == 2) && ((pp & 3) == 1 || (pp & 3) == 2)) ? 2 : 1;
        if (slot < acc + wdt) { part = slot - acc; break; }
        acc += wdt;
    }
    if (pp_out) *pp_out = pp;
    if (part_out) *part_out = part;
    const int py = pp >> 2, px = pp & 3;
    const bool ymid = py == 1 || py == 2, xmid = px == 1 || px == 2;
    if (ymid && xmid) return part;
    if (!ymid && xmid) return py == 0 ? 0 : 1;
    if (ymid && !xmid) return px == 0 ? 2 : 3;
    return py == 0 ? 0 : 1;
}

template <int STAGES>
__global__ __launch_bounds__(512, 2) void gemm_nt_sp_kernel(const NtSpParams p) {
    extern __shared__ __attribute__((aligned(16))) char smem[];
    constexpr int ST = 51200;
    auto slot_base = [&](int t, int kind) __attribute__((always_inline)) {
        const int koff = kind == 0 ? 0 : (kind == 3 ? 9216 : (kind == 1 ? 18432 : 34816));
        return smem + (STAGES == 2 ? (t & 1) : (t % 3)) * ST + koff;
    };
    const int tid = threadIdx.x, lane = tid & 63;
    const int wid = __builtin_amdgcn_readfirstlane(tid >> 6);
    const int wr = wid >> 2, wc = wid & 3;
    int tm, pp, nhalf;
    {
        const int x = blockIdx.x & 7, jj = blockIdx.x >> 3;
        const int seq = jj >> 5, w = jj & 31;
        const int period = seq >> 2, n = seq & 3, y = x & 3;
        int gsel, centre, idx;
        if (x < 4) { gsel = n >> 1; centre = n == 0; idx = n == 0 ? y : (n == 1 ? 8 + y : (n == 2 ? y : 4 + y)); }
        else { gsel = n >> 1; centre = n == 2; idx = n == 0 ? y : (n == 1 ? 4 + y : (n == 2 ? y : 8 + y)); }
        const int G = 2 * period + gsel;
        if (G * 16 >= p.tiles_m) return;
        pp = centre ? (5 + (idx & 1) + 4 * (idx >> 1)) : (idx < 5 ? idx : (idx == 5 ? 7 : (idx == 6 ? 8 : idx + 4)));
        tm = G * 16 + (w >> 1);
        nhalf = w & 1;
        if (tm >= p.tiles_m) return;
    }
    const bool is_centre = ((pp >> 2) == 1 || (pp >> 2) == 2) && ((pp & 3) == 1 || (pp & 3) == 2);
    const int slot = pp + (pp > 5) + (pp > 6) + (pp > 9) + (pp > 10);
    const int set = nt_sp_slot_set(slot);
    const int m0 = tm * 256;

    const int arow = wid * 16 + (lane >> 2);
    const int achunk = (lane & 3) ^ ((arow >> 2) & 3);
    const u16* const a_set = p.Ac + ((long)set * p.entries + m0) * 1024;
    int a_voff[2];
#pragma unroll
    for (int h = 0; h < 2; ++h) a_voff[h] = (((arow >> 6) * 128 + h * 64 + (arow & 63)) * 1024 + achunk * 8) * 2;
    const unsigned* const i_blk = p.Ic + ((long)(set * p.tiles_m + tm) * 2) * 32 * 256;
    const u16* const b_blk = p.B + (long)slot * 512 * 2048 + (long)(nhalf * 256) * 2048;
    const int lrow = lane >> 3, cpos = lane & 7;
    int b_voff[2][2];
#pragma unroll
    for (int q = 0; q < 2; ++q) {
        const int r = (wid * 2 + q) * 8 + lrow;
        const int chunk = (cpos ^ ((r >> 1) & 7)) << 3;
#pragma unroll
        for (int h = 0; h < 2; ++h) b_voff[h][q] = (((r >> 5) * 64 + h * 32 + (r & 31)) * 2048 + chunk) * 2;
    }
    const long a_pass = (long)p.entries * 1024, i_pass = (long)p.tiles_m * 2 * 32 * 256, b_pass = 512L * 2048;
    auto stage = [&](int kind, int t) __attribute__((always_inline)) {
        char* base = slot_base(t, kind);
        const int pass = t >> 5, tt = t & 31;
        if (kind == 0 || kind == 3) {
            const int h = kind ? 1 : 0;
            buf_load_lds16(a_set + pass * a_pass, a_voff[h], tt << 6, base + wid * 1024);
            if (wid == h) buf_load_lds16(i_blk + pass * i_pass, lane << 4, (h * 32 + tt) << 10, base + 8192);
        } else {
            buf_load_lds16(b_blk + pass * b_pass, b_voff[kind - 1][0], tt << 7, base + wid * 2048);
            buf_load_lds16(b_blk + pass * b_pass, b_voff[kind - 1][1], tt << 7, base + wid * 2048 + 1024);
        }
    };

    const int l31 = lane & 31, kh = lane >> 5;
    s16x8 af[2][2];
    unsigned ai[2];
    s16x8 bfr[2][2][2];
    auto read_a = [&](int h, int par) __attribute__((always_inline)) {
        const char* base = slot_base(par, h ? 3 : 0);
#pragma unroll
        for (int i = 0; i < 2; ++i) {
            const int r = wr * 64 + i * 32 + l31;
#pragma unroll
            for (int s = 0; s < 2; ++s)
                af[i][s] = *reinterpret_cast<const s16x8*>(base + r * 64 + (((2 * s + kh) ^ ((r >> 2) & 3)) << 4));
            ai[i] = *reinterpret_cast<const unsigned*>(base + 8192 + kh * 512 + r * 4);
        }
    };
    const int b_rd = (wc * 32 + l31) * 128, bsw = (l31 >> 1) & 7;
    auto read_b = [&](int par) __attribute__((always_inline)) {
#pragma unroll
        for (int h = 0; h < 2; ++h) {
            const char* base = slot_base(par, 1 + h) + b_rd;
#pragma unroll
            for (int s = 0; s < 2; ++s)
#pragma unroll
                for (int c = 0; c < 2; ++c)
                    bfr[h][s][c] = *reinterpret_cast<const s16x8*>(base + (((4 * s + 2 * c + kh) ^ bsw) << 4));
        }
    };

    f32x16 acc[4][2];
#pragma unroll
    for (int i = 0; i < 4; ++i)
#pragma unroll
        for (int j = 0; j < 2; ++j)
#pragma unroll
            for (int r = 0; r < 16; ++r) acc[i][j][r] = 0.f;
    auto mm = [&](int a, int s, int i, int j) __attribute__((always_inline)) {
        const bf16x8_sp av = __builtin_bit_cast(bf16x8_sp, af[i][s]);
        const s16x16_sp_t bw = __builtin_shufflevector(bfr[j][s][0], bfr[j][s][1], 0, 1, 2, 3, 4, 5, 6, 7, 8, 9, 10, 11, 12, 13, 14, 15);
        const bf16x16_sp bv = __builtin_bit_cast(bf16x16_sp, bw);
        if (s == 0) acc[2 * a + i][j] = __builtin_amdgcn_smfmac_f32_32x32x32_bf16(av, bv, acc[2 * a + i][j], (int)ai[i], 0, 0);
        else acc[2 * a + i][j] = __builtin_amdgcn_smfmac_f32_32x32x32_bf16(av, bv, acc[2 * a + i][j], (int)ai[i], 0, 1);
    };
    auto half = [&](int a) __attribute__((always_inline)) {
        __builtin_amdgcn_sched_barrier(0);
#pragma unroll
        for (int s = 0; s < 2; ++s)
#pragma unroll
            for (int i = 0; i < 2; ++i)
#pragma unroll
                for (int j = 0; j < 2; ++j) mm(a, s, i, j);
        SGC_PP_BARRIER();
    };

    const int nk = is_centre ? 64 : 32;
    if constexpr (STAGES == 2) {
        stage(0, 0); stage(1, 0); stage(2, 0); stage(3, 0);
        stage(0, 1); stage(1, 1); stage(2, 1);
        if (wid == 0) SGC_WAIT_VM(6); else SGC_WAIT_VM(5);
    } else {
        stage(0, 0); stage(1, 0); stage(2, 0); stage(3, 0);
        stage(0, 1); stage(1, 1); stage(2, 1); stage(3, 1);
        stage(0, 2); stage(1, 2); stage(2, 2);
        if (wid == 0) SGC_WAIT_VM(13); else if (wid == 1) SGC_WAIT_VM(12); else SGC_WAIT_VM(11);
    }
    __builtin_amdgcn_s_barrier();
    if (wr == 1) __builtin_amdgcn_s_barrier();
    auto close = [&](bool steady) __attribute__((always_inline)) {
        if (!steady) SGC_WAIT_VM(0);
        else if (STAGES == 2) { if (wid < 2) SGC_WAIT_VM(7); else SGC_WAIT_VM(6); }
        else { if (wid < 2) SGC_WAIT_VM(14); else SGC_WAIT_VM(12); }
        SGC_WAIT_LGKM0();
        SGC_PP_BARRIER();
    };
    auto tile = [&](int it, int par, auto steady_c) __attribute__((always_inline)) {
        constexpr bool STEADY = decltype(steady_c)::value;
        read_a(0, par); read_b(par);
        if (it + STAGES - 1 < nk) stage(3, it + STAGES - 1);
        close(STEADY);
        half(0);
        read_a(1, par);
        if (STEADY) { stage(0, it + STAGES); stage(1, it + STAGES); stage(2, it + STAGES); }
        close(STEADY);
        half(1);
    };
    int it = 0;
#pragma unroll 1
    for (; it + STAGES < nk; ++it) tile(it, it, std::true_type{});
#pragma unroll 1
    for (; it < nk; ++it) tile(it, it, std::false_type{});
    if (wr == 0) __builtin_amdgcn_s_barrier();

    NtParams q{};
    q.C = p.C; q.M = p.entries; q.ldc = 16 * 512; q.bias = nullptr;
    nt_epilogue_store16<ELEM_BF16>(q, acc, m0, pp * 512 + nhalf * 256, wr, wc, lane, wid, smem);
}

__global__ __launch_bounds__(256) void nt_sp_weights_kernel(const float* __restrict__ w, u16* __restrict__ B) {
    const int slot = blockIdx.y;
    int pp, part;
    const int set = nt_sp_slot_set(slot, &pp, &part);
    const int py = pp >> 2, px = pp & 3;
    const int q0 = set == 0 ? 0 : (set == 1 ? 2 : (set == 2 ? 0 : 1)), q1 = set == 0 ? 1 : (set == 1 ? 3 : (set == 2 ? 2 : 3));
    int tap[2];
#pragma unroll
    for (int j = 0; j < 2; ++j) {
        const int q = j ? q1 : q0;
        const int ky = py - (q >> 1), kx = px - (q & 1);
        tap[j] = (ky >= 0 && ky <= 2 && kx >= 0 && kx <= 2) ? ky * 3 + kx : -1;
    }
    for (long i = (long)blockIdx.x * 256 + threadIdx.x; i < 512L * 1024; i += (long)gridDim.x * 256) {
        const int n = (int)(i >> 10), c = (int)(i & 1023);
        const float* src = w + ((long)c * 512 + n) * 9;
        const unsigned lo = tap[0] >= 0 ? f32_to_bf16_bits(src[tap[0]]) : 0u;
        const unsigned hi = tap[1] >= 0 ? f32_to_bf16_bits(src[tap[1]]) : 0u;
        reinterpret_cast<unsigned*>(B)[((long)slot * 512 + n) * 1024 + c] = lo | (hi << 16);
    }
}

__global__ __launch_bounds__(256) void nt_sp_pack_kernel(const u16* __restrict__ dywm, const unsigned char* __restrict__ am,
                                                         const int* __restrict__ gather, const int* __restrict__ dest, int n_sparse,
                                                         u16* __restrict__ Ac, unsigned* __restrict__ Ic, float* __restrict__ bias_part) {
    extern __shared__ __attribute__((aligned(16))) char smem[];
    unsigned* sidx = reinterpret_cast<unsigned*>(smem);
    const int lane = threadIdx.x & 63, wv = threadIdx.x >> 6;
    const int tiles_m = n_sparse >> 8, n_groups = n_sparse >> 6;
    float bs[16];
#pragma unroll
    for (int k = 0; k < 16; ++k) bs[k] = 0.f;
    for (int grp = blockIdx.x; grp < n_groups; grp += gridDim.x) {
        for (int wi = wv; wi < 64; wi += 4) {
            const int e = grp * 64 + wi;
            const long row = gather[e], drow = dest ? (long)dest[e] : row;
            uint4 v[2];
            v[0] = *reinterpret_cast<const uint4*>(dywm + drow * 1024 + lane * 16);
            v[1] = *reinterpret_cast<const uint4*>(dywm + drow * 1024 + lane * 16 + 8);
            const uint4 cd = *reinterpret_cast<const uint4*>(am + row * 1024 + lane * 16);
            const u16* vh = reinterpret_cast<const u16*>(v);
            const unsigned cw[4] = {cd.x, cd.y, cd.z, cd.w};
            const unsigned vw[8] = {v[0].x, v[0].y, v[0].z, v[0].w, v[1].x, v[1].y, v[1].z, v[1].w};
            unsigned eq[4][4];
#pragma unroll
            for (int q = 0; q < 4; ++q)
#pragma unroll
                for (int d = 0; d < 4; ++d) {
                    const unsigned x = cw[d] ^ (0x01010101u * (unsigned)q);
                    eq[q][d] = (~(x + 0x7f7f7f7fu) >> 7) & 0x01010101u;
                }
#pragma unroll
            for (int d = 0; d < 4; ++d) {
                const unsigned live = eq[0][d] | eq[1][d] | eq[2][d] | eq[3][d];
#pragma unroll
                for (int b = 0; b < 4; ++b)
                    if ((live >> (8 * b)) & 1u) bs[4 * d + b] += bf16_bits_to_f32(vh[4 * d + b]);
            }
#pragma unroll
            for (int set = 0; set < 4; ++set) {
                const int q0 = set == 0 ? 0 : (set == 1 ? 2 : (set == 2 ? 0 : 1)), q1 = set == 0 ? 1 : (set == 1 ? 3 : (set == 2 ? 2 : 3));
                unsigned ow[8];
                unsigned jb[4];
#pragma unroll
                for (int d = 0; d < 4; ++d) {
                    const unsigned in = (eq[q0][d] | eq[q1][d]) * 0xffu;
                    ow[2 * d] = vw[2 * d] & __builtin_amdgcn_perm(0u, in, 0x01010000u);
                    ow[2 * d + 1] = vw[2 * d + 1] & __builtin_amdgcn_perm(0u, in, 0x03030202u);
                    jb[d] = (eq[q1][d] * 0x01041040u) >> 24;
                }
                const unsigned bits0 = 0x8888u | jb[0] | (jb[1] << 8), bits1 = 0x8888u | jb[2] | (jb[3] << 8);
                u16* dst = Ac + ((long)set * n_sparse + e) * 1024 + lane * 16;
                *reinterpret_cast<uint4*>(dst) = make_uint4(ow[0], ow[1], ow[2], ow[3]);
                *reinterpret_cast<uint4*>(dst + 8) = make_uint4(ow[4], ow[5], ow[6], ow[7]);
                const unsigned mine = bits0 | (bits1 << 16);
                const unsigned other = __shfl_xor(mine, 1);
                if (!(lane & 1)) {
                    const int t = lane >> 1;
                    unsigned* ib = sidx + ((set * 32 + t) * 2) * 64 + wi;
                    ib[0] = (mine & 0xffffu) | (other << 16);
                    ib[64] = (mine >> 16) | (other & 0xffff0000u);
                }
            }
        }
        __syncthreads();
        {
            const int e0 = grp * 64, tm = e0 >> 8, el = e0 & 255;
            const int h = (el >> 6) & 1, r0 = (el >> 7) * 64;
            for (int i = threadIdx.x; i < 4 * 32 * 2 * 64; i += 256) {
                const int rr = i & 63, line = i >> 6;
                const int set = line >> 6, t = (line >> 1) & 31, ha = line & 1;
                Ic[(((((long)(set * tiles_m + tm) * 2 + h) * 32 + t) * 2 + ha) * 128) + r0 + rr] = sidx[i];
            }
        }
        __syncthreads();
    }
    if (bias_part) {
        float* red = reinterpret_cast<float*>(smem);
#pragma unroll
        for (int k = 0; k < 16; ++k) red[wv * 1024 + lane * 16 + k] = bs[k];
        __syncthreads();
        for (int c = threadIdx.x; c < 1024; c += 256)
            bias_part[(long)blockIdx.x * 1024 + c] = (red[c] + red[1024 + c]) + (red[2048 + c] + red[3072 + c]);
    }
}

static int launch_gemm_nt_sp(NtSpParams p, hipStream_t stream) {
    constexpr int LDS = 3 * 51200;
    if (p.entries <= 0) return SGC_OK;
    if (p.entries & 255) return SGC_ERR_ARG;
    p.tiles_m = p.entries >> 8;
    auto kern = gemm_nt_sp_kernel<2>;
    (void)hipFuncSetAttribute(reinterpret_cast<const void*>(kern), hipFuncAttributeMaxDynamicSharedMemorySize, LDS);
    const int groups = (p.tiles_m + 15) >> 4, periods = (groups + 1) >> 1;
    const unsigned grid = (unsigned)(periods * 4 * 8 * 32);
    SGC_LAUNCH(kern, dim3(grid), dim3(512), LDS, stream, p);
    SGC_CHECK_LAUNCH();
    return SGC_OK;
}

extern "C" {

int sgc_windows_dgrad_sparse_weights(const float* conv3_weight, void* w3sp, void* stream) {
    SGC_LAUNCH(nt_sp_weights_kernel, dim3(512, 20), dim3(256), 0, (hipStream_t)stream, conv3_weight, (u16*)w3sp);
    SGC_CHECK_LAUNCH();
    return SGC_OK;
}

int sgc_windows_dgrad_sparse_pack(const void* dywm, const unsigned char* argmax, const int* gather, const int* dest, int n_sparse,
                                  void* pack_a, void* pack_i, float* bias_part, int* n_parts, void* stream) {
    if (n_parts) *n_parts = 0;
    if (n_sparse <= 0) return SGC_OK;
    if (n_sparse & 255) return SGC_ERR_ARG;
    const int blocks = grid_cap_sp(n_sparse >> 6, 1, 768);
    if (n_parts && bias_part) *n_parts = blocks;
    (void)hipFuncSetAttribute(reinterpret_cast<const void*>(nt_sp_pack_kernel), hipFuncAttributeMaxDynamicSharedMemorySize, 65536);
    SGC_LAUNCH(nt_sp_pack_kernel, dim3(blocks), dim3(256), 65536, (hipStream_t)stream, (const u16*)dywm, argmax, gather, dest, n_sparse, (u16*)pack_a,
               (unsigned*)pack_i, bias_part);
    SGC_CHECK_LAUNCH();
    return SGC_OK;
}

int sgc_windows_dgrad_patches_sparse(const void* pack_a, const void* pack_i, int n_sparse, const void* w3sp, void* patch, void* stream) {
    if (n_sparse <= 0) return SGC_OK;
    if (n_sparse & 255) return SGC_ERR_ARG;
    NtSpParams p{};
    p.Ac = (const u16*)pack_a; p.Ic = (const unsigned*)pack_i; p.B = (const u16*)w3sp; p.C = (u16*)patch; p.entries = n_sparse;
    return launch_gemm_nt_sp(p, (hipStream_t)stream);
}

}
```

Measured before the change: 849,800 pairs/s.

## Switch NT GEMM kernels from 32x32x16 to 16x16x32 MFMA fragments

Replaces the 32x32 MFMA accumulator tiles in the NT GEMM and conv/pool kernels with 16x16x32 MFMA fragments. This reworks the LDS read offsets, swizzles, fragment-to-row mapping (including a halo mapping for the conv kernel) and all epilogues to match. The sparse kernel keeps the old 32x32 layout through a copied epilogue. The aim is better MFMA throughput or fewer LDS reads per FLOP on MI355X, at the cost of more MFMA instructions and different register pressure.

```diff
diff --git a/include/sgc_relhead.h b/include/sgc_relhead.h
--- a/include/sgc_relhead.h
+++ b/include/sgc_relhead.h
@@ -350,6 +350,7 @@
 int sgc_dbg_gemm_tn(int elem, const void* A, const void* B, float* C, int M, int N, int K, long lda, long ldb, int splits, int* slabs, void* stream);
 int sgc_dbg_conv_tn(int elem, const void* A, const void* B, float* C, int M, int n_img, int lgS, int Cin, int splits, int* slabs, void* stream);
 int sgc_dbg_tr_probe(const int* addr, short* out, void* stream);
+int sgc_dbg_mfma16_probe(int elem, const void* a, const void* b, float* c, void* stream);
 int sgc_dbg_mfma_rate(float* out, int blocks, int iters, int mode, void* stream);
 int sgc_dbg_smfmac_probe(const void* a, const void* b, const int* idx, float* c, int abid, void* stream);
 
diff --git a/scene_graph_commonsense_amd/csrc/capi_debug.hip b/scene_graph_commonsense_amd/csrc/capi_debug.hip
--- a/scene_graph_commonsense_amd/csrc/capi_debug.hip
+++ b/scene_graph_commonsense_amd/csrc/capi_debug.hip
@@ -63,6 +63,20 @@
     return SGC_OK;
 }
 
+__global__ void mfma16_probe_kernel(const u16* a, const u16* b, float* c, int elem) {
+    const int l = threadIdx.x;
+    s16x8 av, bv;
+    for (int i = 0; i < 8; ++i) { av[i] = (short)a[l * 8 + i]; bv[i] = (short)b[l * 8 + i]; }
+    f32x4 acc = {0.f, 0.f, 0.f, 0.f};
+    acc = elem == ELEM_F16 ? mfma16<ELEM_F16>(av, bv, acc) : mfma16<ELEM_BF16>(av, bv, acc);
+    for (int r = 0; r < 4; ++r) c[l * 4 + r] = acc[r];
+}
+int sgc_dbg_mfma16_probe(int elem, const void* a, const void* b, float* c, void* stream) {
+    SGC_LAUNCH(mfma16_probe_kernel, dim3(1), dim3(64), 0, (hipStream_t)stream, (const u16*)a, (const u16*)b, c, elem);
+    SGC_CHECK_LAUNCH();
+    return SGC_OK;
+}
+
 __global__ void smfmac_probe_kernel(const u16* a, const u16* b, const int* idx, float* c, int abid) {
     typedef __bf16 bf16x8_t __attribute__((ext_vector_type(8)));
     typedef __bf16 bf16x16_t __attribute__((ext_vector_type(16)));
diff --git a/scene_graph_commonsense_amd/csrc/gemm_nt.h b/scene_graph_commonsense_amd/csrc/gemm_nt.h
--- a/scene_graph_commonsense_amd/csrc/gemm_nt.h
+++ b/scene_graph_commonsense_amd/csrc/gemm_nt.h
@@ -41,6 +41,21 @@
     }
 }
 
+template <int ELEM>
+__device__ __forceinline__ f32x4 mfma16(s16x8 a, s16x8 b, f32x4 c) {
+    if constexpr (ELEM == ELEM_F16) {
+        return __builtin_amdgcn_mfma_f32_16x16x32_f16(__builtin_bit_cast(f16x8, a), __builtin_bit_cast(f16x8, b), c, 0, 0, 0);
+    } else {
+        return __builtin_amdgcn_mfma_f32_16x16x32_bf16(__builtin_bit_cast(bf16x8, a), __builtin_bit_cast(bf16x8, b), c, 0, 0, 0);
+    }
+}
+
+template <bool HALO>
+__device__ __forceinline__ int frag_row(int i, int r) {
+    if constexpr (HALO) return (i >> 1) * 32 + ((2 * (r >> 2) + (i & 1)) << 2) + (r & 3);
+    else return i * 16 + r;
+}
+
 __device__ __forceinline__ long conv_row_base(int m, int lgS, int Cin) {
     const int S = 1 << lgS;
     const int img = m >> (2 * lgS);
@@ -51,50 +66,47 @@
     return ((long)(img * (S + 2) + y) * (S + 2) + x) * Cin;
 }
 
-template <int ELEM, int EPI, int TM, int TN, bool GATHER = false>
-__device__ __forceinline__ void nt_epilogue(const NtParams& p, f32x16 (&acc)[TM][TN], int m0, int n0, int wr, int wc, int lane, int m_limit = -1) {
+template <int ELEM, int EPI, int FM, int FN, bool GATHER = false, bool HALO = false>
+__device__ __forceinline__ void nt_epilogue(const NtParams& p, f32x4 (&acc)[FM][FN], int m0, int n0, int wr, int wc, int lane, int m_limit = -1) {
     const int M = GATHER ? m_limit : p.M;
-    const int h = lane >> 5, cl = lane & 31;
-#pragma unroll
-    for (int i = 0; i < TM; ++i) {
-#pragma unroll
-        for (int j = 0; j < TN; ++j) {
-            const int col = n0 + wc * TN * 32 + j * 32 + cl;
-            const int rbase = m0 + wr * TM * 32 + i * 32;
+    const int g = lane >> 4, cl = lane & 15;
+#pragma unroll
+    for (int i = 0; i < FM; ++i) {
+#pragma unroll
+        for (int j = 0; j < FN; ++j) {
+            const int col = n0 + wc * FN * 16 + j * 16 + cl;
+            const int rbase = m0 + wr * FM * 16 + frag_row<HALO>(i, 4 * g);
             const float bias = p.bias ? p.bias[col] : 0.f;
             if constexpr (EPI == EPI_POOL) {
                 u16* out = reinterpret_cast<u16*>(p.C);
-#pragma unroll
-                for (int w = 0; w < 4; ++w) {
-                    float v = acc[i][j][4 * w];
-                    int am = 0;
-#pragma unroll
-                    for (int q = 1; q < 4; ++q) {
-                        const float t = acc[i][j][4 * w + q];
-                        if (t > v) { v = t; am = q; }
+                float v = acc[i][j][0];
+                int am = 0;
+#pragma unroll
+                for (int q = 1; q < 4; ++q) {
+                    const float t = acc[i][j][q];
+                    if (t > v) { v = t; am = q; }
+                }
+                v += bias;
+                const int prow = rbase >> 2;
+                if (prow * 4 < M) {
+                    long arow = prow, yrow = prow;
+                    if constexpr (GATHER) {
+                        arow = p.gather[prow]; yrow = p.dest ? p.dest[prow] : arow;
+                        if (p.raw && prow >= p.raw_first) {
+#pragma unroll
+                            for (int q = 0; q < 4; ++q) p.raw[((long)(prow - p.raw_first) * 4 + q) * p.ldc + col] = acc[i][j][q];
+                        }
                     }
-                    v += bias;
-                    const int prow = (rbase >> 2) + 2 * w + h;
-                    if (prow * 4 < M) {
-                        long arow = prow, yrow = prow;
-                        if constexpr (GATHER) {
-                            arow = p.gather[prow]; yrow = p.dest ? p.dest[prow] : arow;
-                            if (p.raw && prow >= p.raw_first) {
-#pragma unroll
-                                for (int q = 0; q < 4; ++q) p.raw[((long)(prow - p.raw_first) * 4 + q) * p.ldc + col] = acc[i][j][4 * w + q];
-                            }
-                        }
-                        else if (p.wm_goff) yrow = p.wm_goff[prow & 63] + (prow >> 6);
-                        if (!(v > 0.f)) { v = 0.f; am = 4; }
-                        out[yrow * p.ldc + col] = to_elem<ELEM>(v);
-                        if (p.C2) p.C2[yrow * p.ldc + col] = f32_to_bf16_bits(v);
-                        if (p.argmax) p.argmax[arow * p.ldc + col] = (unsigned char)am;
-                    }
+                    else if (p.wm_goff) yrow = p.wm_goff[prow & 63] + (prow >> 6);
+                    if (!(v > 0.f)) { v = 0.f; am = 4; }
+                    out[yrow * p.ldc + col] = to_elem<ELEM>(v);
+                    if (p.C2) p.C2[yrow * p.ldc + col] = f32_to_bf16_bits(v);
+                    if (p.argmax) p.argmax[arow * p.ldc + col] = (unsigned char)am;
                 }
             } else {
 #pragma unroll
-                for (int r = 0; r < 16; ++r) {
-                    const int row = rbase + (r & 3) + 8 * (r >> 2) + 4 * h;
+                for (int r = 0; r < 4; ++r) {
+                    const int row = rbase + r;
                     if (row >= M) continue;
                     float v = acc[i][j][r];
                     long o = (long)row * p.ldc + col;
@@ -125,36 +137,33 @@
     }
 }
 
-__device__ __forceinline__ void nt_epilogue_f32t(const NtParams& p, f32x16 (&acc)[4][2], int m0, int n0, int wr, int wc, int lane) {
-    const int h = lane >> 5, cl = lane & 31;
+__device__ __forceinline__ void nt_epilogue_f32t(const NtParams& p, f32x4 (&acc)[8][4], int m0, int n0, int wr, int wc, int lane) {
+    const int g = lane >> 4, cl = lane & 15;
     float* out = reinterpret_cast<float*>(p.C);
     if (!out) return;
     const int g_first = p.Cx ? p.wm_goff[p.tile_group[m0 >> 8]] + p.x_first : 0;
 #pragma unroll
-    for (int i = 0; i < 4; ++i) {
-        const int row = m0 + wr * 128 + i * 32 + cl;
+    for (int i = 0; i < 8; ++i) {
+        const int row = m0 + wr * 128 + i * 16 + cl;
         if (row >= p.M) continue;
         const bool xrow = p.Cx && row >= g_first;
 #pragma unroll
-        for (int j = 0; j < 2; ++j) {
-#pragma unroll
-            for (int rq = 0; rq < 4; ++rq) {
-                const int col = n0 + wc * 64 + j * 32 + 8 * rq + 4 * h;
-                f32x4 v = {acc[i][j][4 * rq], acc[i][j][4 * rq + 1], acc[i][j][4 * rq + 2], acc[i][j][4 * rq + 3]};
-                if (p.bias) {
-                    const f32x4 b = *reinterpret_cast<const f32x4*>(p.bias + col);
-                    v += b;
-                }
-                if (xrow) {
-                    uint2 hv;
-                    hv.x = (unsigned)f32_to_f16_bits(v[0]) | ((unsigned)f32_to_f16_bits(v[1]) << 16);
-                    hv.y = (unsigned)f32_to_f16_bits(v[2]) | ((unsigned)f32_to_f16_bits(v[3]) << 16);
-                    *reinterpret_cast<uint2*>(p.Cx + (long)row * p.N + col) = hv;
-                    continue;
-                }
-                f32x4* dst = reinterpret_cast<f32x4*>(out + (long)row * p.ldc + col);
-                *dst = v;
-            }
+        for (int j = 0; j < 4; ++j) {
+            const int col = n0 + wc * 64 + j * 16 + 4 * g;
+            f32x4 v = acc[i][j];
+            if (p.bias) {
+                const f32x4 b = *reinterpret_cast<const f32x4*>(p.bias + col);
+                v += b;
+            }
+            if (xrow) {
+                uint2 hv;
+                hv.x = (unsigned)f32_to_f16_bits(v[0]) | ((unsigned)f32_to_f16_bits(v[1]) << 16);
+                hv.y = (unsigned)f32_to_f16_bits(v[2]) | ((unsigned)f32_to_f16_bits(v[3]) << 16);
+                *reinterpret_cast<uint2*>(p.Cx + (long)row * p.N + col) = hv;
+                continue;
+            }
+            f32x4* dst = reinterpret_cast<f32x4*>(out + (long)row * p.ldc + col);
+            *dst = v;
         }
     }
 }
@@ -186,31 +195,31 @@
 
 constexpr int EPI_LDS_PITCH = 128;
 constexpr int EPI_LDS_BYTES = 8 * 128 * EPI_LDS_PITCH;
-template <int ELEM, bool MASK = false>
-__device__ __forceinline__ void nt_epilogue_store16(const NtParams& p, f32x16 (&acc)[4][2], int m0, int n0, int wr, int wc, int lane,
+template <int ELEM, bool MASK = false, bool HALO = false>
+__device__ __forceinline__ void nt_epilogue_store16(const NtParams& p, f32x4 (&acc)[8][4], int m0, int n0, int wr, int wc, int lane,
                                                     int wid, char* smem) {
     __syncthreads();
     char* reg = smem + wid * (128 * EPI_LDS_PITCH);
-    const int h = lane >> 5, cl = lane & 31;
+    const int g = lane >> 4, cl = lane & 15;
     const bool odd = cl & 1;
-#pragma unroll
-    for (int i = 0; i < 4; ++i) {
-#pragma unroll
-        for (int j = 0; j < 2; ++j) {
-            const int col = n0 + wc * 64 + j * 32 + cl;
+    constexpr int QB = HALO ? 8 : 4;
+#pragma unroll
+    for (int i = 0; i < 8; ++i) {
+#pragma unroll
+        for (int j = 0; j < 4; ++j) {
+            const int col = n0 + wc * 64 + j * 16 + cl;
             const float bias = p.bias ? p.bias[col] : 0.f;
 #pragma unroll
-            for (int rp = 0; rp < 8; ++rp) {
+            for (int rp = 0; rp < 2; ++rp) {
                 float v0 = acc[i][j][2 * rp] + bias, v1 = acc[i][j][2 * rp + 1] + bias;
                 if constexpr (MASK) { v0 *= p.scale; v1 *= p.scale; }
                 const float recv = __shfl_xor(odd ? v0 : v1, 1);
-                const int r0 = ((2 * rp) & 3) + 8 * ((2 * rp) >> 2) + 4 * h;
                 const float flo = odd ? recv : v0, fhi = odd ? v1 : recv;
                 unsigned packed;
                 if constexpr (ELEM == ELEM_BF16) packed = f32x2_to_bf16x2_bits(flo, fhi);
                 else packed = (unsigned)to_elem<ELEM>(flo) | ((unsigned)to_elem<ELEM>(fhi) << 16);
-                const int row = i * 32 + r0 + (odd ? 1 : 0);
-                *reinterpret_cast<unsigned*>(reg + row * EPI_LDS_PITCH + (((j * 32 + (cl & ~1)) * 2) ^ ((row & 1) << 6))) = packed;
+                const int row = frag_row<HALO>(i, 4 * g + 2 * rp) + (odd ? 1 : 0);
+                *reinterpret_cast<unsigned*>(reg + row * EPI_LDS_PITCH + (((j * 16 + (cl & ~1)) * 2) ^ ((row & 1) << 6) ^ ((row & QB) ? 32 : 0))) = packed;
             }
         }
     }
@@ -220,7 +229,7 @@
 #pragma unroll
     for (int it = 0; it < 16; ++it) {
         const int rowl = it * 8 + rsub;
-        uint4 v = *reinterpret_cast<const uint4*>(reg + rowl * EPI_LDS_PITCH + ((c8 * 16) ^ ((rowl & 1) << 6)));
+        uint4 v = *reinterpret_cast<const uint4*>(reg + rowl * EPI_LDS_PITCH + ((c8 * 16) ^ ((rowl & 1) << 6) ^ ((rowl & QB) ? 32 : 0)));
         const int row = m0 + wr * 128 + rowl;
         if (row < p.M) {
             const long o = (long)row * p.ldc + n0 + wc * 64 + c8 * 8;
@@ -296,25 +305,16 @@
     };
 
     const int wr = wid / WC, wc = wid % WC;
-    const int kh = lane >> 5;
-    int a_off[TM], a_sw[TM], b_off[TN], b_sw[TN];
-#pragma unroll
-    for (int i = 0; i < TM; ++i) {
-        const int ra = wr * TM * 32 + i * 32 + (lane & 31);
-        a_off[i] = ra * 128; a_sw[i] = (ra >> 1) & 7;
-    }
-#pragma unroll
-    for (int i = 0; i < TN; ++i) {
-        const int rb = wc * TN * 32 + i * 32 + (lane & 31);
-        b_off[i] = rb * 128; b_sw[i] = (rb >> 1) & 7;
-    }
-    f32x16 acc[TM][TN];
-#pragma unroll
-    for (int i = 0; i < TM; ++i)
-#pragma unroll
-        for (int j = 0; j < TN; ++j)
-#pragma unroll
-            for (int r = 0; r < 16; ++r) acc[i][j][r] = 0.f;
+    const int kg = lane >> 4, sw = ((lane & 15) >> 1) & 7;
+    constexpr int FM = 2 * TM, FN = 2 * TN;
+    const int a_rd = (wr * TM * 32 + (lane & 15)) * 128, b_rd = (wc * TN * 32 + (lane & 15)) * 128;
+    f32x4 acc[FM][FN];
+#pragma unroll
+    for (int i = 0; i < FM; ++i)
+#pragma unroll
+        for (int j = 0; j < FN; ++j)
+#pragma unroll
+            for (int r = 0; r < 4; ++r) acc[i][j][r] = 0.f;
 
     const int nk = p.K >> 6;
     stage(0, 0);
@@ -325,25 +325,25 @@
         const char* ab = smem + (kt & 1) * BUF_BYTES;
         const char* bb = ab + A_BYTES;
 #pragma unroll
-        for (int ks = 0; ks < 4; ++ks) {
-            const int c = ks * 2 + kh;
-            s16x8 af[TM], bf[TN];
-#pragma unroll
-            for (int i = 0; i < TM; ++i) af[i] = *reinterpret_cast<const s16x8*>(ab + a_off[i] + ((c ^ a_sw[i]) << 4));
-#pragma unroll
-            for (int i = 0; i < TN; ++i) bf[i] = *reinterpret_cast<const s16x8*>(bb + b_off[i] + ((c ^ b_sw[i]) << 4));
-#pragma unroll
-            for (int i = 0; i < TM; ++i)
-#pragma unroll
-                for (int j = 0; j < TN; ++j) acc[i][j] = mfma32<ELEM>(af[i], bf[j], acc[i][j]);
+        for (int ks = 0; ks < 2; ++ks) {
+            const int ko = ((ks * 4 + kg) ^ sw) << 4;
+            s16x8 af[FM], bf[FN];
+#pragma unroll
+            for (int i = 0; i < FM; ++i) af[i] = *reinterpret_cast<const s16x8*>(ab + a_rd + i * 2048 + ko);
+#pragma unroll
+            for (int i = 0; i < FN; ++i) bf[i] = *reinterpret_cast<const s16x8*>(bb + b_rd + i * 2048 + ko);
+#pragma unroll
+            for (int i = 0; i < FM; ++i)
+#pragma unroll
+                for (int j = 0; j < FN; ++j) acc[i][j] = mfma16<ELEM>(af[i], bf[j], acc[i][j]);
         }
     }
 
     if constexpr (EPI == EPI_STORE && TM == 4 && TN == 2 && WR * WC == 8) {
         if (p.epi_lds) { nt_epilogue_store16<ELEM>(p, acc, m0, n0, wr, wc, lane, wid, smem); return; }
     }
-    if constexpr (AMODE == AMODE_CONV_GATHER) nt_epilogue<ELEM, EPI, TM, TN, true>(p, acc, m0, n0, wr, wc, lane, Mlim);
-    else nt_epilogue<ELEM, EPI, TM, TN>(p, acc, m0, n0, wr, wc, lane);
+    if constexpr (AMODE == AMODE_CONV_GATHER) nt_epilogue<ELEM, EPI, FM, FN, true>(p, acc, m0, n0, wr, wc, lane, Mlim);
+    else nt_epilogue<ELEM, EPI, FM, FN>(p, acc, m0, n0, wr, wc, lane);
 }
 
 template <int ELEM, int AMODE, int EPI, int WR, int WC, int TM, int TN>
diff --git a/scene_graph_commonsense_amd/csrc/gemm_nt_pp.h b/scene_graph_commonsense_amd/csrc/gemm_nt_pp.h
--- a/scene_graph_commonsense_amd/csrc/gemm_nt_pp.h
+++ b/scene_graph_commonsense_amd/csrc/gemm_nt_pp.h
@@ -39,8 +39,8 @@
     return tm < tiles_m && w < gm * wn;
 }
 
-template <int ELEM, bool GATHER>
-__device__ __forceinline__ void nt_epilogue_pool16(const NtParams& p, f32x16 (&acc)[4][2], int m0, int n0, int wr, int wc, int lane,
+template <int ELEM, bool GATHER, bool HALO = false>
+__device__ __forceinline__ void nt_epilogue_pool16(const NtParams& p, f32x4 (&acc)[8][4], int m0, int n0, int wr, int wc, int lane,
                                                    int wid, char* smem, int m_limit);
 template <int ELEM, int EPI, int ACG = 0, int SEG = 0>
 __global__ __launch_bounds__(512, 2) void gemm_nt_pp_kernel(const NtParams p) {
@@ -142,45 +142,45 @@
         buf_load_lds16(g, voff[kind][1], soff, base + 1024);
     };
 
-    const int l31 = lane & 31, kh = lane >> 5, sw = (l31 >> 1) & 7;
-    int ko[4];
-#pragma unroll
-    for (int ks = 0; ks < 4; ++ks) ko[ks] = ((ks * 2 + kh) ^ sw) << 4;
-    const int a_rd = (wr * 64 + l31) * 128, b_rd = (wc * 32 + l31) * 128;
-    s16x8 af[2][4], bf[2][4];
+    const int l15 = lane & 15, kg = lane >> 4, sw = (l15 >> 1) & 7;
+    int ko[2];
+#pragma unroll
+    for (int ks = 0; ks < 2; ++ks) ko[ks] = ((ks * 4 + kg) ^ sw) << 4;
+    const int a_rd = (wr * 64 + l15) * 128, b_rd = (wc * 32 + l15) * 128;
+    s16x8 af[4][2], bf[4][2];
     auto read_a = [&](int h, int par) __attribute__((always_inline)) {
         const char* base = smem + ((par << 2) + (h ? 3 : 0)) * HT + a_rd;
 #pragma unroll
-        for (int i = 0; i < 2; ++i)
-#pragma unroll
-            for (int ks = 0; ks < 4; ++ks) af[i][ks] = *reinterpret_cast<const s16x8*>(base + i * 4096 + ko[ks]);
+        for (int i = 0; i < 4; ++i)
+#pragma unroll
+            for (int ks = 0; ks < 2; ++ks) af[i][ks] = *reinterpret_cast<const s16x8*>(base + i * 2048 + ko[ks]);
     };
     auto read_b = [&](int par) __attribute__((always_inline)) {
 #pragma unroll
-        for (int h = 0; h < 2; ++h) {
-            const char* base = smem + ((par << 2) + 1 + h) * HT + b_rd;
-#pragma unroll
-            for (int ks = 0; ks < 4; ++ks) bf[h][ks] = *reinterpret_cast<const s16x8*>(base + ko[ks]);
-        }
-    };
-
-    f32x16 acc[4][2];
-#pragma unroll
-    for (int i = 0; i < 4; ++i)
-#pragma unroll
-        for (int j = 0; j < 2; ++j)
-#pragma unroll
-            for (int r = 0; r < 16; ++r) acc[i][j][r] = 0.f;
+        for (int j = 0; j < 4; ++j) {
+            const char* base = smem + ((par << 2) + 1 + (j >> 1)) * HT + b_rd + (j & 1) * 2048;
+#pragma unroll
+            for (int ks = 0; ks < 2; ++ks) bf[j][ks] = *reinterpret_cast<const s16x8*>(base + ko[ks]);
+        }
+    };
+
+    f32x4 acc[8][4];
+#pragma unroll
+    for (int i = 0; i < 8; ++i)
+#pragma unroll
+        for (int j = 0; j < 4; ++j)
+#pragma unroll
+            for (int r = 0; r < 4; ++r) acc[i][j][r] = 0.f;
     auto half = [&](int a) __attribute__((always_inline)) {
         __builtin_amdgcn_sched_barrier(0);
 #pragma unroll
-        for (int ks = 0; ks < 4; ++ks)
-#pragma unroll
-            for (int i = 0; i < 2; ++i)
-#pragma unroll
-                for (int j = 0; j < 2; ++j) {
-                    if constexpr (EPI == EPI_STORE_F32T) acc[2 * a + i][j] = mfma32<ELEM>(bf[j][ks], af[i][ks], acc[2 * a + i][j]);
-                    else acc[2 * a + i][j] = mfma32<ELEM>(af[i][ks], bf[j][ks], acc[2 * a + i][j]);
+        for (int ks = 0; ks < 2; ++ks)
+#pragma unroll
+            for (int i = 0; i < 4; ++i)
+#pragma unroll
+                for (int j = 0; j < 4; ++j) {
+                    if constexpr (EPI == EPI_STORE_F32T) acc[4 * a + i][j] = mfma16<ELEM>(bf[j][ks], af[i][ks], acc[4 * a + i][j]);
+                    else acc[4 * a + i][j] = mfma16<ELEM>(af[i][ks], bf[j][ks], acc[4 * a + i][j]);
                 }
         SGC_PP_BARRIER();
     };
@@ -229,10 +229,10 @@
     }
     else if constexpr (ACG && EPI == EPI_POOL) {
         if (p.epi_lds) nt_epilogue_pool16<ELEM, true>(p, acc, m0, n0, wr, wc, lane, wid, smem, Mlim);
-        else nt_epilogue<ELEM, EPI, 4, 2, true>(p, acc, m0, n0, wr, wc, lane, Mlim);
-    }
-    else if constexpr (ACG) nt_epilogue<ELEM, EPI, 4, 2, true>(p, acc, m0, n0, wr, wc, lane, Mlim);
-    else nt_epilogue<ELEM, EPI, 4, 2>(p, acc, m0, n0, wr, wc, lane);
+        else nt_epilogue<ELEM, EPI, 8, 4, true>(p, acc, m0, n0, wr, wc, lane, Mlim);
+    }
+    else if constexpr (ACG) nt_epilogue<ELEM, EPI, 8, 4, true>(p, acc, m0, n0, wr, wc, lane, Mlim);
+    else nt_epilogue<ELEM, EPI, 8, 4>(p, acc, m0, n0, wr, wc, lane);
 }
 
 template <int ELEM, int EPI>
@@ -282,43 +282,42 @@
 
 constexpr int POOL_EPI_PY = 128, POOL_EPI_PA = 64;
 constexpr int POOL_EPI_WAVE_BYTES = 32 * POOL_EPI_PY * 2 + 32 * POOL_EPI_PA;
-template <int ELEM, bool GATHER>
-__device__ __forceinline__ void nt_epilogue_pool16(const NtParams& p, f32x16 (&acc)[4][2], int m0, int n0, int wr, int wc, int lane,
+template <int ELEM, bool GATHER, bool HALO>
+__device__ __forceinline__ void nt_epilogue_pool16(const NtParams& p, f32x4 (&acc)[8][4], int m0, int n0, int wr, int wc, int lane,
                                                    int wid, char* smem, int m_limit) {
     __syncthreads();
     char* ty = smem + wid * POOL_EPI_WAVE_BYTES;
     char* tb = ty + 32 * POOL_EPI_PY;
     char* ta = tb + 32 * POOL_EPI_PY;
-    const int h = lane >> 5, cl = lane & 31;
-#pragma unroll
-    for (int i = 0; i < 4; ++i)
-#pragma unroll
-        for (int j = 0; j < 2; ++j) {
-            const int colw = j * 32 + cl;
+    const int g = lane >> 4, cl = lane & 15;
+    constexpr int RB = HALO ? 1 : 0;
+#pragma unroll
+    for (int i = 0; i < 8; ++i)
+#pragma unroll
+        for (int j = 0; j < 4; ++j) {
+            const int colw = j * 16 + cl;
             const float bias = p.bias ? p.bias[n0 + wc * 64 + colw] : 0.f;
-#pragma unroll
-            for (int w = 0; w < 4; ++w) {
-                float v = acc[i][j][4 * w];
-                int am = 0;
-#pragma unroll
-                for (int q = 1; q < 4; ++q) {
-                    const float t = acc[i][j][4 * w + q];
-                    if (t > v) { v = t; am = q; }
+            float v = acc[i][j][0];
+            int am = 0;
+#pragma unroll
+            for (int q = 1; q < 4; ++q) {
+                const float t = acc[i][j][q];
+                if (t > v) { v = t; am = q; }
+            }
+            v += bias;
+            if (!(v > 0.f)) { v = 0.f; am = 4; }
+            const int row = frag_row<HALO>(i, 4 * g) >> 2;
+            if constexpr (GATHER) {
+                const int prow = (m0 >> 2) + wr * 32 + row;
+                if (p.raw && prow >= p.raw_first && prow * 4 < m_limit) {
+#pragma unroll
+                    for (int q = 0; q < 4; ++q) p.raw[((long)(prow - p.raw_first) * 4 + q) * p.ldc + n0 + wc * 64 + colw] = acc[i][j][q];
                 }
-                v += bias;
-                if (!(v > 0.f)) { v = 0.f; am = 4; }
-                const int row = i * 8 + 2 * w + h;
-                if constexpr (GATHER) {
-                    const int prow = (m0 >> 2) + wr * 32 + row;
-                    if (p.raw && prow >= p.raw_first && prow * 4 < m_limit) {
-#pragma unroll
-                        for (int q = 0; q < 4; ++q) p.raw[((long)(prow - p.raw_first) * 4 + q) * p.ldc + n0 + wc * 64 + colw] = acc[i][j][4 * w + q];
-                    }
-                }
-                *reinterpret_cast<u16*>(ty + row * POOL_EPI_PY + colw * 2) = to_elem<ELEM>(v);
-                if (p.C2) *reinterpret_cast<u16*>(tb + row * POOL_EPI_PY + colw * 2) = f32_to_bf16_bits(v);
-                if (p.argmax) *reinterpret_cast<unsigned char*>(ta + row * POOL_EPI_PA + colw) = (unsigned char)am;
-            }
+            }
+            const int yo = (colw * 2) ^ (((row >> RB) & 1) << 5);
+            *reinterpret_cast<u16*>(ty + row * POOL_EPI_PY + yo) = to_elem<ELEM>(v);
+            if (p.C2) *reinterpret_cast<u16*>(tb + row * POOL_EPI_PY + yo) = f32_to_bf16_bits(v);
+            if (p.argmax) *reinterpret_cast<unsigned char*>(ta + row * POOL_EPI_PA + colw) = (unsigned char)am;
         }
     __builtin_amdgcn_wave_barrier();
     const long prow0 = ((long)m0 >> 2) + wr * 32;
@@ -333,8 +332,9 @@
             orow = p.dest ? p.dest[orow] : p.gather[orow];
         } else if (p.wm_goff) orow = p.wm_goff[orow & 63] + (orow >> 6);
         const long o = orow * p.ldc + n0 + wc * 64 + c8 * 8;
-        *reinterpret_cast<uint4*>(out + o) = *reinterpret_cast<const uint4*>(ty + row * POOL_EPI_PY + c8 * 16);
-        if (p.C2) *reinterpret_cast<uint4*>(p.C2 + o) = *reinterpret_cast<const uint4*>(tb + row * POOL_EPI_PY + c8 * 16);
+        const int yo = (c8 * 16) ^ (((row >> RB) & 1) << 5);
+        *reinterpret_cast<uint4*>(out + o) = *reinterpret_cast<const uint4*>(ty + row * POOL_EPI_PY + yo);
+        if (p.C2) *reinterpret_cast<uint4*>(p.C2 + o) = *reinterpret_cast<const uint4*>(tb + row * POOL_EPI_PY + yo);
     }
     if (p.argmax) {
         const int c4 = lane & 3, r16 = lane >> 2;
@@ -443,57 +443,50 @@
         }
     };
 
-    const int l31 = lane & 31, kh = lane >> 5;
-    int a_row[4], a_px[4], a_py[4];
-#pragma unroll
-    for (int i = 0; i < 4; ++i) {
-        const int m = wr * 128 + i * 32 + l31;
-        const int W = m >> 2, q = m & 3;
-        a_py[i] = 2 * (W >> 3) + (q >> 1);
-        a_px[i] = 2 * (W & 7) + (q & 1);
-        a_row[i] = a_py[i] * 18 + a_px[i];
-    }
-    const int bsw = (l31 >> 1) & 7;
-    int bko[4];
-#pragma unroll
-    for (int ks = 0; ks < 4; ++ks) bko[ks] = ((ks * 2 + kh) ^ bsw) << 4;
-    const int b_rd = (wc * 32 + l31) * 128;
-    s16x8 af[2][4], bf[2][4];
+    const int l15 = lane & 15, kg = lane >> 4;
+    const int a_py0 = 8 * wr + ((l15 >> 1) & 1), a_px0 = 4 * (l15 >> 2) + (l15 & 1);
+    const int a_row0 = a_py0 * 18 + a_px0;
+    const int bsw = (l15 >> 1) & 7;
+    int bko[2];
+#pragma unroll
+    for (int ks = 0; ks < 2; ++ks) bko[ks] = ((ks * 4 + kg) ^ bsw) << 4;
+    const int b_rd = (wc * 32 + l15) * 128;
+    s16x8 af[4][2], bf[4][2];
     auto read_a = [&](int h, int cc, int ky, int kx) __attribute__((always_inline)) {
         const char* ab = abuf0 + (cc & 1) * A_BYTES;
 #pragma unroll
-        for (int i = 0; i < 2; ++i) {
-            const int ii = 2 * h + i;
-            const char* rowp = ab + (a_row[ii] + ky * 18 + kx) * 128;
-            const int f = (((a_px[ii] + kx) >> 1) + 4 * ((a_py[ii] + ky) & 1)) & 7;
-#pragma unroll
-            for (int ks = 0; ks < 4; ++ks) af[i][ks] = *reinterpret_cast<const s16x8*>(rowp + (((ks * 2 + kh) ^ f) << 4));
+        for (int i = 0; i < 4; ++i) {
+            const int ii = 4 * h + i;
+            const char* rowp = ab + (a_row0 + ((ii >> 1) * 2 + ky) * 18 + (ii & 1) * 2 + kx) * 128;
+            const int f = (((a_px0 + (ii & 1) * 2 + kx) >> 1) + 4 * ((a_py0 + ky) & 1)) & 7;
+#pragma unroll
+            for (int ks = 0; ks < 2; ++ks) af[i][ks] = *reinterpret_cast<const s16x8*>(rowp + (((ks * 4 + kg) ^ f) << 4));
         }
     };
     auto read_b = [&](int step) __attribute__((always_inline)) {
 #pragma unroll
-        for (int h = 0; h < 2; ++h) {
-            const char* base = bbuf0 + ((step & 1) * 2 + h) * HT + b_rd;
-#pragma unroll
-            for (int ks = 0; ks < 4; ++ks) bf[h][ks] = *reinterpret_cast<const s16x8*>(base + bko[ks]);
-        }
-    };
-
-    f32x16 acc[4][2];
-#pragma unroll
-    for (int i = 0; i < 4; ++i)
-#pragma unroll
-        for (int j = 0; j < 2; ++j)
-#pragma unroll
-            for (int r = 0; r < 16; ++r) acc[i][j][r] = 0.f;
+        for (int j = 0; j < 4; ++j) {
+            const char* base = bbuf0 + ((step & 1) * 2 + (j >> 1)) * HT + b_rd + (j & 1) * 2048;
+#pragma unroll
+            for (int ks = 0; ks < 2; ++ks) bf[j][ks] = *reinterpret_cast<const s16x8*>(base + bko[ks]);
+        }
+    };
+
+    f32x4 acc[8][4];
+#pragma unroll
+    for (int i = 0; i < 8; ++i)
+#pragma unroll
+        for (int j = 0; j < 4; ++j)
+#pragma unroll
+            for (int r = 0; r < 4; ++r) acc[i][j][r] = 0.f;
     auto half = [&](int a) __attribute__((always_inline)) {
         __builtin_amdgcn_sched_barrier(0);
 #pragma unroll
-        for (int ks = 0; ks < 4; ++ks)
-#pragma unroll
-            for (int i = 0; i < 2; ++i)
-#pragma unroll
-                for (int j = 0; j < 2; ++j) acc[2 * a + i][j] = mfma32<ELEM>(af[i][ks], bf[j][ks], acc[2 * a + i][j]);
+        for (int ks = 0; ks < 2; ++ks)
+#pragma unroll
+            for (int i = 0; i < 4; ++i)
+#pragma unroll
+                for (int j = 0; j < 4; ++j) acc[4 * a + i][j] = mfma16<ELEM>(af[i][ks], bf[j][ks], acc[4 * a + i][j]);
         SGC_PP_BARRIER();
     };
 
@@ -562,12 +555,12 @@
     if (wr == 0) __builtin_amdgcn_s_barrier();
 
     if constexpr (EPI == EPI_STORE) {
-        if (p.epi_lds) { nt_epilogue_store16<ELEM>(p, acc, m0, n0, wr, wc, lane, wid, smem); return; }
+        if (p.epi_lds) { nt_epilogue_store16<ELEM, false, true>(p, acc, m0, n0, wr, wc, lane, wid, smem); return; }
     }
     if constexpr (EPI == EPI_POOL) {
-        if (p.epi_lds) { nt_epilogue_pool16<ELEM, false>(p, acc, m0, n0, wr, wc, lane, wid, smem, 0); return; }
-    }
-    nt_epilogue<ELEM, EPI, 4, 2>(p, acc, m0, n0, wr, wc, lane);
+        if (p.epi_lds) { nt_epilogue_pool16<ELEM, false, true>(p, acc, m0, n0, wr, wc, lane, wid, smem, 0); return; }
+    }
+    nt_epilogue<ELEM, EPI, 8, 4, false, true>(p, acc, m0, n0, wr, wc, lane);
 }
 
 template <int ELEM, int EPI>
diff --git a/scene_graph_commonsense_amd/csrc/kernels_dgrad_sp.hip b/scene_graph_commonsense_amd/csrc/kernels_dgrad_sp.hip
--- a/scene_graph_commonsense_amd/csrc/kernels_dgrad_sp.hip
+++ b/scene_graph_commonsense_amd/csrc/kernels_dgrad_sp.hip
@@ -38,6 +38,58 @@
     if (ymid && !xmid) return px == 0 ? 2 : 3;
     return py == 0 ? 0 : 1;
 }
+
+template <int ELEM, bool MASK = false>
+__device__ __forceinline__ void sp_epilogue_store16(const NtParams& p, f32x16 (&acc)[4][2], int m0, int n0, int wr, int wc, int lane,
+                                                    int wid, char* smem) {
+    __syncthreads();
+    char* reg = smem + wid * (128 * EPI_LDS_PITCH);
+    const int h = lane >> 5, cl = lane & 31;
+    const bool odd = cl & 1;
+#pragma unroll
+    for (int i = 0; i < 4; ++i) {
+#pragma unroll
+        for (int j = 0; j < 2; ++j) {
+            const int col = n0 + wc * 64 + j * 32 + cl;
+            const float bias = p.bias ? p.bias[col] : 0.f;
+#pragma unroll
+            for (int rp = 0; rp < 8; ++rp) {
+                float v0 = acc[i][j][2 * rp] + bias, v1 = acc[i][j][2 * rp + 1] + bias;
+                if constexpr (MASK) { v0 *= p.scale; v1 *= p.scale; }
+                const float recv = __shfl_xor(odd ? v0 : v1, 1);
+                const int r0 = ((2 * rp) & 3) + 8 * ((2 * rp) >> 2) + 4 * h;
+                const float flo = odd ? recv : v0, fhi = odd ? v1 : recv;
+                unsigned packed;
+                if constexpr (ELEM == ELEM_BF16) packed = f32x2_to_bf16x2_bits(flo, fhi);
+                else packed = (unsigned)to_elem<ELEM>(flo) | ((unsigned)to_elem<ELEM>(fhi) << 16);
+                const int row = i * 32 + r0 + (odd ? 1 : 0);
+                *reinterpret_cast<unsigned*>(reg + row * EPI_LDS_PITCH + (((j * 32 + (cl & ~1)) * 2) ^ ((row & 1) << 6))) = packed;
+            }
+        }
+    }
+    __builtin_amdgcn_wave_barrier();
+    u16* out = reinterpret_cast<u16*>(p.C);
+    const int c8 = lane & 7, rsub = lane >> 3;
+#pragma unroll
+    for (int it = 0; it < 16; ++it) {
+        const int rowl = it * 8 + rsub;
+        uint4 v = *reinterpret_cast<const uint4*>(reg + rowl * EPI_LDS_PITCH + ((c8 * 16) ^ ((rowl & 1) << 6)));
+        const int row = m0 + wr * 128 + rowl;
+        if (row < p.M) {
+            const long o = (long)row * p.ldc + n0 + wc * 64 + c8 * 8;
+            if constexpr (MASK) {
+                const uint4 f = *reinterpret_cast<const uint4*>(p.mask_src + o);
+                const u16* fh = reinterpret_cast<const u16*>(&f);
+                u16* vh = reinterpret_cast<u16*>(&v);
+#pragma unroll
+                for (int k = 0; k < 8; ++k)
+                    if (!(from_elem<ELEM_F16>(fh[k]) > 0.f)) vh[k] = 0;
+            }
+            *reinterpret_cast<uint4*>(out + o) = v;
+        }
+    }
+}
+
 
 template <int STAGES>
 __global__ __launch_bounds__(512, 2) void gemm_nt_sp_kernel(const NtSpParams p) {
@@ -194,7 +246,7 @@
 
     NtParams q{};
     q.C = p.C; q.M = p.entries; q.ldc = 16 * 512; q.bias = nullptr;
-    nt_epilogue_store16<ELEM_BF16>(q, acc, m0, pp * 512 + nhalf * 256, wr, wc, lane, wid, smem);
+    sp_epilogue_store16<ELEM_BF16>(q, acc, m0, pp * 512 + nhalf * 256, wr, wc, lane, wid, smem);
 }
 
 __global__ __launch_bounds__(256) void nt_sp_weights_kernel(const float* __restrict__ w, u16* __restrict__ B) {
```

Result: faster. 869,000 pairs/s (median of 6 runs) (+2.3%).
